# Wionerlol/MultimodalEmotionRecognition

Hardware: AMD Instinct MI355X
Metric: 3s-clip train steps/sec (B=32, xattn fusion) at 1/2/4/8 MI355X (higher is better)
Workload: dtype bf16; 1 GPU; ResNet18 + WavLM-base (frozen) + xattn fusion train step (fwd+bwd+Adam); per_gpu_batch=32, global_batch=32, frames=8, image=112, audio_samples=48000, parallelism=dp1

## Files before the change

### include/mer.h

```cpp
#ifndef MER_H_
#define MER_H_

#define MER_BN_STAT_PARTS 64
#define MER_BN_STAT_ROWS(M) (((M) + 63) / 64 + 64)
#define MER_BN_RED_ROWS(M) (((M) + 63) / 64 + 4 + 64)
#define MER_BN_RED_WS_ROWS 576

#ifdef __cplusplus
extern "C" {
#endif


int mer_gemm_f32(int M, int N, int K, const void* A, int a_dtype, long sam, long sak, long bsa, const void* B,
                 int b_dtype, long sbk, long sbn, long bsb, float* C, long ldc, long bsc, const float* bias, int beta,
                 int act, int splitk, int batch, float* workspace, void* stream);

#define MER_COLSUM_WS_FLOATS(M, N) ((long)(((M) + 15) / 16) * (N))
int mer_colsum_f32(int M, int N, const float* X, long ldx, float* out, float* workspace, void* stream);

int mer_mha_fwd(int B, int H, int Lq, int Lk, int dh, const float* Q, long ldq, const float* K, long ldk,
                const float* V, long ldv, const float* bias, float* O, long ldo, float* P, float scale, float drop_p,
                const unsigned long long* seed, unsigned long long site, void* stream);

int mer_mha_bwd(int B, int H, int Lq, int Lk, int dh, const float* Q, long ldq, const float* K, long ldk,
// ... 32 lines not shown
int mer_softmax_dropout_bwd(int B, int H, int h, int Lq, int Lk, const float* P, const float* dPp, float* dS,
                            float* Pd, float p, const unsigned long long* seed, unsigned long long site, void* stream);
int mer_softmax_dropout_fwd(int B, int H, int h, int Lq, int Lk, const float* S, float scale, float* P, float* Pd,
                            float p, const unsigned long long* seed, unsigned long long site, void* stream);

int mer_cross_entropy(int B, int C, const float* logits, const long long* labels, float label_smoothing, int late,
                      float* loss, float* dlogits, long long* preds, void* stream);

int mer_rng_advance(unsigned long long* state, void* stream);

int mer_scale_dev(long n, const float* x, const float* s, float* y, void* stream);

int mer_dropout_inplace(int rows, int cols, float* x, long ldx, float p, const unsigned long long* seed, unsigned long long site, void* stream);

int mer_relu_dropout_bwd(int rows, int cols, float* dy, long lddy, const float* y, long ldy, float p,
                         const unsigned long long* seed, unsigned long long site, void* stream);

int mer_gate_mix_fwd(int B, int D, const float* z, const float* v, long ldv, const float* a, long lda, float* out,
                     float* g_out, void* stream);
int mer_gate_mix_bwd(int B, int D, const float* g, const float* v, long ldv, const float* a, long lda,
                     const float* dout, float* dz, float* dv, long lddv, float* da, long ldda, void* stream);

int mer_token_bias_fwd(int B, int Lq, int Lk, const float* qt, const float* qp, const float* kt, const float* kp,
                       const float* scale, float* out, void* stream);
int mer_token_bias_bwd(int B, int Lq, int Lk, const float* qt, const float* qp, const float* kt, const float* kp,
                       const float* scale, const float* dbias, float* dqt, float* dkt, float* dqp, float* dkp,
                       float* dscale_part, void* stream);

int mer_softmax_avg_fwd(int B, int C, const float* za, const float* zv, float* out, float* pa, float* pv, void* stream);
int mer_softmax_avg_bwd(int B, int C, const float* pa, const float* pv, const float* dout, float* da, float* dv,
                        void* stream);

int mer_vec_sum(int n, const float* x, float* out, int accumulate, void* stream);

int mer_adam_step(long n, float* p, const float* g, float* m, float* v, float lr, float b1, float b2, float eps,
                  float wd, int step, float grad_scale, void* stream);


int mer_gemm_bf16(int M, int N, int K, const void* A, long a_gstride, long a_rstride, int a_rpg, const void* W,
                  long ldw, void* C, int c_dtype, long ldc, const float* bias, const void* R, long ldr, int act,
                  void* stream);

int mer_gemm_bf16_ex(int M, int N, int K, const void* A, long a_gstride, long a_rstride, int a_rpg, const void* W,
                     long ldw, void* C, int c_dtype, long ldc, const float* bias, const void* R, long ldr, int act,
                     int variant, void* stream);

int mer_posconv_gemm_bf16(int B, int L, int C_total, int groups, int taps, int pad, const void* X, long ldx,
                          const void* Wp, void* out, int out_dtype, long ldo, const float* bias, const void* R,
                          long ldr, int act, int variant, void* stream);

int mer_wavlm_conv0_gn_gelu(int B, int S, int Lout, const float* wav, const float* w0, const float* gamma,
                            const float* beta, float eps, float* workspace, void* out, void* stream);

int mer_layernorm(int rows, int d, const void* x, int x_dtype, long ldx, const float* gamma, const float* beta,
                  float eps, void* y, int y_dtype, long ldy, void* stream);

int mer_wavlm_attention(int B, int L, int H, const void* qkv, long ldqkv, const void* x, long ldx, const float* gate_w,
                        const float* gate_b, const float* gate_const, const float* rel_emb, const int* bucket,
                        void* out, long ldo, float scale, void* stream);

int mer_permute3_bf16(int n0, int n1, int n2, const float* src, long s0, long s1, long s2, const float* scale,
                      void* dst, void* stream);

int mer_weightnorm_scale(int n01, int taps, const float* v, const float* g, float* scale, void* stream);

int mer_cast_bf16(long n, const float* x, void* y, void* stream);


int mer_gemm_bf16_tr(int M, int N, int K, const void* A, long a_gstride, long a_rstride, int a_rpg, const void* W,
                     long ldw, void* C, int c_dtype, long ldc, const float* bias, const void* R, long ldr, int act,
                     float drop_p, const unsigned long long* seed, unsigned long long site, const long long* skip_mask,
                     int skip_bit, int variant, void* stream);

int mer_layernorm_tr(int rows, int d, const void* x, int x_dtype, long ldx, const float* gamma, const float* beta,
                     float eps, void* y, int y_dtype, long ldy, float drop_p, const unsigned long long* seed,
                     unsigned long long site, const long long* skip_mask, int skip_bit, void* stream);

int mer_wavlm_attention_tr(int B, int L, int H, const void* qkv, long ldqkv, const void* x, long ldx,
                           const float* gate_w, const float* gate_b, const float* gate_const, const float* rel_emb,
                           const int* bucket, void* out, long ldo, float scale, float drop_p,
                           const unsigned long long* seed, unsigned long long site, const long long* skip_mask,
                           int skip_bit, void* stream);

int mer_wavlm_time_mask(int B, int L, int D, void* h, long ldh, const float* embed, float mask_prob, int mask_len,
                        int min_masks, const unsigned long long* seed, unsigned long long site, unsigned char* mask_out,
                        void* stream);

int mer_bf16_convert(long n, const void* x, void* y, int y_dtype, void* stream);


int mer_ln_bwd(int rows, int d, const float* dy_a, const float* dy_b, const float* dy_c, const float* x,
               const float* gamma, float eps, float* dx32, void* dx16, float* part, void* stream);

int mer_fold_rows(int parts, int n, const float* part, long ldp, float* out, float* workspace, void* stream);

int mer_colpart(int rows, int cols, const void* x, int x_dtype, long ldx, float* part, void* stream);

int mer_gelu_bf16(long n, const void* z, void* f, void* stream);

int mer_gelu_bwd(int rows, int cols, const float* df, const void* z, void* dz, float* part, void* stream);

int mer_linear_wgrad(int M, int N, int K, const void* x, const void* dy, long ldy, float* dw, int splits,
                     float* workspace, void* stream);

int mer_wavlm_attention_bwd(int B, int L, int H, const void* qkv, long ldqkv, const void* x, long ldx,
                            const void* dout, long ldo, const float* gate_w, const float* gate_b,
                            const float* gate_const, const float* tbl, float scale, void* scratch,
                            void* dqkv, long lddq, float* dx_gate, long lddxg, float* gate_part, void* stream);
int mer_wavlm_attention_bwd_tr(int B, int L, int H, const void* qkv, long ldqkv, const void* x, long ldx,
                               const void* dout, long ldo, const float* gate_w, const float* gate_b,
                               const float* gate_const, const float* tbl, float scale, void* scratch,
                               void* dqkv, long lddq, float* dx_gate, long lddxg, float* gate_part, float drop_p,
                               const unsigned long long* seed, unsigned long long site, void* stream);
int mer_dropout_rows(int rows, int cols, const void* x, int x_dtype, long ldx, float* y32, long ldy32, void* y16,
                     long ldy16, float p, const unsigned long long* seed, unsigned long long site, void* stream);
int mer_wavlm_attention_bwd_kp(int L);

int mer_transpose_bf16(int rows, int cols, const void* src, long lds, void* dst, long ldd, void* stream);


int mer_frames_resize_normalize(int N, int H0, int W0, const void* frames, long frame_stride, int S, float mean0,
                                float mean1, float mean2, float std0, float std1, float std2, float* out, void* stream);

int mer_frames_resize_u8(int N, int H0, int W0, const void* frames, long frame_stride, int S, void* out, void* stream);
int mer_frames_augment_normalize(int N, int S, int T, const void* frames_u8, const float* clip_params,
                                 const unsigned long long* clip_seeds, const float* ztable, float mean0, float mean1,
                                 float mean2, float std0, float std1, float std2, float* out, void* stream);

int mer_wav_pad_crop(int B, int target, const float* packed, const long long* offsets, const long long* lengths,
                     float* out, void* stream);


int mer_conv_fwd(int N, int H, int W, int C, int K, int R, int S, int stride, int pad, const void* x,
                 const void* w_packed, void* y, float* stats, void* stream);

int mer_conv_fwd_ex(int N, int H, int W, int C, int K, int R, int S, int stride, int pad, const void* x,
                    const void* w_packed, void* y, float* stats, int variant, void* stream);

int mer_conv_dgrad(int N, int H, int W, int C, int K, int R, int S, int stride, int pad, const void* dy,
                   const void* wt_packed, void* dx, const void* residual, const void* residual_mask, void* stream);
int mer_conv_dgrad_ex(int N, int H, int W, int C, int K, int R, int S, int stride, int pad, const void* dy,
                      const void* wt_packed, void* dx, const void* residual, const void* residual_mask, int variant,
                      void* stream);

int mer_conv_dgrad_bnr(int N, int H, int W, int C, int K, int R, int S, int stride, int pad, const void* dy,
                       const void* wt_packed, void* dx, const void* residual, const void* residual_mask,
                       const void* bn_mask, const void* bn_x, const float* bn_ms, float* bn_red, const void* bn_x2,
                       const float* bn_ms2, float* bn_red2, int variant, void* stream);
int mer_conv_dgrad_ds(int N, int H, int W, int C, int K, int R, int S, int stride, int pad, const void* dy,
                      const void* wt_packed, void* dx, const void* residual, const void* residual_mask,
                      const void* bn_mask, const void* bn_x, const float* bn_ms, float* bn_red, const void* bn_x2,
                      const float* bn_ms2, float* bn_red2, const void* ds_dy, const void* ds_wt_packed, int ds_K,
                      int variant, void* stream);

int mer_conv_fwd_rows(int N, int H, int W, int C, int K, int R, int S, int stride, int pad, const void* x,
                      const void* w_packed, int variant);
int mer_conv_dgrad_rows(int N, int H, int W, int C, int K, int R, int S, int stride, int pad, const void* dy,
                        const void* wt_packed, const void* ds_dy, int variant);

int mer_partials_sum(int C, int parts, float* in, float* out, void* stream);
int mer_partials_sum2(int C, int parts, float* in, float* out, float* in2, float* out2, void* stream);

int mer_conv_wgrad(int N, int H, int W, int C, int Creal, int K, int R, int S, int stride, int pad, const void* x,
                   const void* dy, float* dw, int splits, float* workspace, void* stream);
int mer_conv_wgrad_ex(int N, int H, int W, int C, int Creal, int K, int R, int S, int stride, int pad, const void* x,
                      const void* dy, float* dw, int splits, float* workspace, int variant, void* stream);
int mer_conv_wgrad_partials(int N, int H, int W, int C, int K, int R, int S, int stride, int pad, const void* x,
                            const void* dy, int splits, float* workspace, int variant, void* stream);
int mer_wgrad_fold_batch(int n, const long long* rows, void* stream);

int mer_pack_input_nhwc(int N, int C, int H, int W, int Cp, const float* x, void* y, void* stream);
int mer_pack_input_s2d(int N, int C, int H, int W, const float* x, void* y, void* stream);

int mer_pack_conv_weight(int K, int C, int R, int S, int Cp, int transpose, const float* w, void* out, void* stream);

int mer_pack_conv_weights(int n, const long long* desc, long total, void* stream);
int mer_pack_conv_weights_flat(int n, const long long* desc, long total_blocks, void* stream);

int mer_bn_finalize(int C, long M, const float* stats, float eps, float momentum, float* ms, float* rmean,
                    float* rvar, long long* num_batches_tracked, void* stream);
int mer_bn_finalize_rows(int C, long M, int data_rows, const float* stats, float eps, float momentum, float* ms,
                         float* rmean, float* rvar, long long* num_batches_tracked, void* stream);
int mer_bn_finalize_rows2(int C, long M, int data_rows, const float* stats, float* ms, float* rmean, float* rvar,
                          long long* nbt, int C2, long M2, int data_rows2, const float* stats2, float* ms2,
                          float* rmean2, float* rvar2, long long* nbt2, float eps, float momentum, void* stream);

int mer_bn_apply(long M, int C, const void* x, const float* ms, const float* gamma, const float* beta, const void* res,
                 const float* ms2, const float* gamma2, const float* beta2, int relu, void* y, void* stream);

int mer_bn_bwd_reduce(long M, int C, const void* dy, const void* mask, const void* x, const float* ms, float* red,
                      float* workspace, void* stream);

int mer_bn_bwd_apply(long M, int C, const void* dy, const void* mask, const void* x, const float* ms,
                     const float* gamma, const float* red, int batch_stats, void* dx, float* dgamma, float* dbeta,
                     void* stream);
int mer_bn_bwd_apply2(long M, int C, const void* dy, const void* mask, const void* x, const float* ms,
                      const float* gamma, const float* red, const void* x2, const float* ms2, const float* gamma2,
                      const float* red2, int batch_stats, void* dx, void* dx2, float* dgamma, float* dbeta,
                      float* dgamma2, float* dbeta2, void* stream);

int mer_stem_bnrelu_maxpool_fwd(int N, int H, int W, int C, const void* x, const float* ms, const float* gamma,
                                const float* beta, void* y, void* argmax, void* stream);
int mer_stem_pool_bn_bwd(int N, int H, int W, int C, const void* dy, const void* argmax, const void* x,
                         const float* ms, const float* gamma, const float* beta, float* red, int batch_stats,
                         void* dx, float* dgamma, float* dbeta, float* workspace, void* stream);

int mer_maxpool_fwd(int N, int H, int W, int C, const void* x, void* y, void* argmax, void* stream);
int mer_maxpool_bwd(int N, int H, int W, int C, const void* dy, const void* argmax, void* dx, void* stream);

int mer_avgpool_fwd(int N, int HW, int C, const void* x, float* y, void* stream);
int mer_avgpool_bwd(int N, int HW, int C, const float* dy, void* dx, void* stream);


int mer_quant_params(long n, const void* x, int x_dtype, float* partial, int mode, float* qparams, void* stream);

int mer_quantize_weight_s8(int N, int K, const float* w, long ldw, const float* qparams, void* qw, long ldq,
                           int* colsum, void* stream);

int mer_gemm_i8dyn(int M, int N, int K, const void* x, int x_dtype, long ldx, const float* x_qparams, const void* qw,
                   long ldq, const float* w_qparams, const int* colsum, const float* bias, int act, float* out, long ldo,
                   void* stream);

int mer_concat_prior_rows(int B, int L, int d, int pd, int ldo, const float* tok, const float* prior, float* out,
                          void* stream);


int mer_xh_split(int n_items, const long long* desc, void* stream);

int mer_xh_audio_fwd_pair(int M, const float* pair, long ldp, const float* bs, const void* Wa_hi, const void* Wa_lo,
                          const float* ba, const void* Wc_hi, const void* Wc_lo, const float* bq2, const float* bkv1,
                          float* a_s, float* a, float* q2, float* kv1, int Mv, int vdim, const float* vfeat,
                          const void* Wv_hi, const void* Wv_lo, const float* bv, const void* Wq1_hi, const void* Wq1_lo,
                          const float* bq1, float* v, float* q1, void* stream);

int mer_xh_audio_fwd(int M, int S, const void* aseq, int aseq_dtype, long ldas, const void* Ws_hi, const void* Ws_lo,
                     const float* bs, const void* Wa_hi, const void* Wa_lo, const float* ba, const void* Wc_hi,
                     const void* Wc_lo, const float* bq2, const float* bkv1, float* a_s, float* a, float* q2,
                     float* kv1, int Mv, int vdim, const float* vfeat, const void* Wv_hi, const void* Wv_lo,
                     const float* bv, const void* Wq1_hi, const void* Wq1_lo, const float* bq1, float* v, float* q1,
                     void* stream);

int mer_xh_v2a_fwd(int B, int T, int Ta, const float* v, const float* q1, const float* kv1, const void* Wo1_hi,
                   const void* Wo1_lo, const float* bo1, const float* gamma, const float* beta, const void* Wkv2_hi,
                   const void* Wkv2_lo, const float* bkv2, float attn_p, float path_p, const unsigned long long* seed,
                   unsigned long long site_attn, unsigned long long site_path, float scale, float* P1, float* o1,
                   float* s_v, float* mean_v, float* rstd_v, float* v1, float* kv2, float* emb, long ld_emb,
                   const float* bias, void* stream);

int mer_xh_a2v_fwd(int B, int T, int Ta, const float* q2, const float* kv2, const float* a, const void* Wo2_hi,
                   const void* Wo2_lo, const float* bo2, const float* gamma, const float* beta, float attn_p,
                   float path_p, const unsigned long long* seed, unsigned long long site_attn,
                   unsigned long long site_path, float scale, float* P2, float* o2, float* s_a, float* mean_a,
                   float* rstd_a, float* part, const float* bias, void* stream);

int mer_xh_prior_fwd(int B, int T, int Ta, int d, int H1, int PD, const float* v, const float* a, const float* W0,
                     const float* b0, const float* W3, const float* b3, const float* w_vq, const float* b_vq,
                     const float* w_ak, const float* b_ak, const float* w_aq, const float* b_aq, const float* w_vk,
                     const float* b_vk, const float* scale, float drop_p, const unsigned long long* seed,
                     unsigned long long site, float* pg, float* h1, float* prior, float* tt_vq, float* tt_ak,
                     float* tt_aq, float* tt_vk, float* tp_vq, float* tp_ak, float* tp_aq, float* tp_vk,
                     float* v2a_bias, float* a2v_bias, void* stream);

int mer_xh_prior_bwd(int B, int T, int Ta, int d, int H1, int PD, const float* dbias_v2a, const float* dbias_a2v,
                     const float* tt_vq, const float* tt_ak, const float* tt_aq, const float* tt_vk,
                     const float* tp_vq, const float* tp_ak, const float* tp_aq, const float* tp_vk,
                     const float* scale, const float* w_vq, const float* w_ak, const float* w_aq, const float* w_vk,
                     const float* W0, const float* W3, const float* h1, float drop_p, const unsigned long long* seed,
                     unsigned long long site, float* dtt_vq, float* dtt_ak, float* dtt_aq, float* dtt_vk,
                     float* dtp_vq, float* dtp_ak, float* dtp_aq, float* dtp_vk, float* dprior, float* dh1,
                     float* dscale_part, float* dv, float* da, void* stream);

int mer_xh_mlp_fwd(int B, int Ta, int gated, int H1, int C, const float* part, float* emb, const float* W0,
                   const float* b0, const float* W3, const float* b3, const float* Wc, const float* bc, float mlp_p,
                   const unsigned long long* seed, unsigned long long site, float* hsave, float* gsave, float* fsave,
                   float* logits, void* stream);


int mer_xh_mlp_bwd(int B, int C, int H1, int gated, const float* dlogits, const float* emb, const float* h,
                   const float* g, const float* W0, const float* W3, const float* Wc, float mlp_p,
                   const unsigned long long* seed, unsigned long long site, float* dh, float* dz, float* demb,
                   void* stream);

int mer_xh_a2v_bwd(int B, int T, int Ta, const float* demb, const float* s_a, const float* mean_a, const float* rstd_a,
                   const float* gamma, const float* P2, const float* kv2, const float* q2, const void* WoT2_hi,
                   const void* WoT2_lo, float attn_p, float path_p, const unsigned long long* seed,
                   unsigned long long site_attn, unsigned long long site_path, float scale, float* da, float* da2,
                   float* dqkv, float* dkv2_part, float* ln_part, float* dbias, void* stream);

int mer_xh_v2a_bwd(int B, int T, int Ta, const float* dkv2_part, const void* WkvT2_hi, const void* WkvT2_lo,
                   const float* demb, const float* s_v, const float* mean_v, const float* rstd_v, const float* gamma,
                   const void* WoT1_hi, const void* WoT1_lo, const float* P1, const float* kv1, const float* q1,
                   float attn_p, float path_p, const unsigned long long* seed, unsigned long long site_attn,
                   unsigned long long site_path, float scale, float* dkv2, float* dv2, float* dq1, float* dv,
                   float* dqkv, float* ln_part, float* do1, float* dS_heads, float* dbias, void* stream);

int mer_xh_audio_bwd(int M, const float* dqkv, const void* WcT_hi, const void* WcT_lo, const void* WaT_hi,
                     const void* WaT_lo, float* da, float* da_s, int Mv, int vdim, const float* dq1,
                     const void* WqT1_hi, const void* WqT1_lo, const void* WvT_hi, const void* WvT_lo, float* dv,
                     float* dvfeat, void* stream);

int mer_xh_wgrad_ws_floats(int nprob, const long long* table, long long* out);
int mer_xh_wgrad(int nprob, const long long* table, float* ws, long long ws_floats, void* stream);

int mer_clip_align_fwd(int B, int D, const float* a, const float* v, const float* log_scale, float* an, float* vn,
                       float* norms, float* logits, float* loss, void* stream);
int mer_clip_align_bwd(int B, int D, const float* an, const float* vn, const float* norms, const float* logits,
                       const float* log_scale, const float* dloss, float* ws, float* da, float* dv, float* dlog_scale,
                       void* stream);
int mer_add_scaled_scalar(const float* x, const float* y, float w, float* out, void* stream);

#ifdef __cplusplus
}
#endif
#endif
```

### multimodalemotionrecognition_amd/csrc/bn_pool.hip

```cpp
#include "common.h"
#include "mer.h"

typedef __attribute__((ext_vector_type(4))) uint32_t u32x4;

__global__ __launch_bounds__(256) void bn_stat_rows_fold_kernel(int C2, int rows, int per, const float* __restrict__ in,
                                                                float* __restrict__ out) {
  __shared__ float part[4][64];
  const int el = threadIdx.x & 63, pg = threadIdx.x >> 6;
  const int e = blockIdx.x * 64 + el, grp = blockIdx.y;
  const int r0 = grp * per, r1 = min(rows, r0 + per);
  const int ec = e < C2 ? e : C2 - 1;
  const int n = r1 - (r0 + pg) > 0 ? (r1 - (r0 + pg) + 3) / 4 : 0;
  float a0 = 0.f, a1 = 0.f;
  for (int i0 = 0; i0 < n; i0 += 16) {
    float x[16];
#pragma unroll
    for (int i = 0; i < 16; ++i) {
      const int r = r0 + pg + 4 * (i0 + i);
      x[i] = in[(long)(r < r1 ? r : r1 - 1) * C2 + ec];
    }
#pragma unroll
    for (int i = 0; i < 16; i += 2) {
      if (i0 + i < n) a0 += x[i];
      if (i0 + i + 1 < n) a1 += x[i + 1];
// ... 435 lines not shown
  hipLaunchKernelGGL(partials_sum_kernel, dim3((2 * C + 63) / 64), dim3(256), 0, st, C, parts, src, out);
  MER_LAUNCH_CHECK();
}
MER_API int mer_partials_sum(int C, int parts, float* in, float* out, void* stream) {
  if (C <= 0 || parts <= 0) return (int)hipErrorInvalidValue;
  return partials_fold(C, parts, in, out, (hipStream_t)stream);
}

MER_API int mer_partials_sum2(int C, int parts, float* in, float* out, float* in2, float* out2, void* stream) {
  if (C <= 0 || parts <= 0 || !in || !out || !in2 || !out2) return (int)hipErrorInvalidValue;
  hipStream_t st = (hipStream_t)stream;
  if (parts > BN_WIDE_ROWS) {
    const int rc = partials_fold(C, parts, in, out, st);
    return rc ? rc : partials_fold(C, parts, in2, out2, st);
  }
  const dim3 grid((2 * C + 63) / 64, 2);
#define MER_PSUM2(NB) \
  [&] { hipLaunchKernelGGL(partials_sum_wide2_kernel<NB>, grid, dim3(1024), 0, st, 2 * C, parts, in, out, in2, out2); }
  wide_pick(parts, MER_PSUM2(16), MER_PSUM2(32), MER_PSUM2(64));
#undef MER_PSUM2
  MER_LAUNCH_CHECK();
}

template <bool BNMASK>
__global__ __launch_bounds__(256) void bn_bwd_apply_kernel(long M, int C, const bf16_t* dy,
                                                           const bf16_t* __restrict__ mask,
                                                           const bf16_t* __restrict__ x, const float* __restrict__ ms,
                                                           const float* __restrict__ gamma,
                                                           const float* __restrict__ mbeta,
                                                           const float* __restrict__ red, int batch_stats,
                                                           bf16_t* dx, float* __restrict__ dgamma,
                                                           float* __restrict__ dbeta) {
  __shared__ __attribute__((aligned(16))) float coef[5][512];
  const float invM = 1.f / (float)M;
  for (int c = threadIdx.x; c < C; c += 256) {
    if (blockIdx.x == 0) {
      if (dgamma) dgamma[c] += red[2 * c + 1];
      if (dbeta) dbeta[c] += red[2 * c];
    }
    const float mu = ms[2 * c], rs = ms[2 * c + 1], gr = gamma[c] * rs;
    const float a = batch_stats ? red[2 * c] * invM : 0.f;
    const float b = batch_stats ? red[2 * c + 1] * invM : 0.f;
    const float t = gr * b * rs;
    coef[0][c] = gr;
    coef[1][c] = -t;
    coef[2][c] = fmaf(-gr, a, t * mu);
    if (BNMASK) stem_bn_coef(c, ms, gamma, mbeta, coef[3][c], coef[4][c]);
  }
  __syncthreads();
  const long nvec = M * C / 8;
  const long stride = (long)gridDim.x * blockDim.x;
  const long tid0 = blockIdx.x * (long)blockDim.x + threadIdx.x;
  const int c0 = (int)(tid0 % (C / 8)) * 8;
  float k1[8], k2[8], k0[8], msc[8], msh[8];
#pragma unroll
  for (int i = 0; i < 8; ++i) {
    k1[i] = coef[0][c0 + i];
    k2[i] = coef[1][c0 + i];
    k0[i] = coef[2][c0 + i];
    msc[i] = BNMASK ? coef[3][c0 + i] : 0.f;
    msh[i] = BNMASK ? coef[4][c0 + i] : 0.f;
  }
  auto one = [&](const u32x4& gv, const u32x4& xv, const u32x4& mv) -> u32x4 {
    const bf16_t* gh = reinterpret_cast<const bf16_t*>(&gv);
    const bf16_t* xh = reinterpret_cast<const bf16_t*>(&xv);
    const bf16_t* mh = reinterpret_cast<const bf16_t*>(&mv);
    u32x4 ov;
    bf16_t* oh = reinterpret_cast<bf16_t*>(&ov);
#pragma unroll
    for (int i = 0; i < 8; ++i) {
      const bool live = BNMASK ? bf2f(f2bf(fmaxf(bf2f(xh[i]) * msc[i] + msh[i], 0.f))) > 0.f
                               : (!mask || bf2f(mh[i]) > 0.f);
      const float g = live ? bf2f(gh[i]) : 0.f;
      oh[i] = f2bf(fmaf(k1[i], g, fmaf(k2[i], bf2f(xh[i]), k0[i])));
    }
    return ov;
  };
  const u32x4 one16 = {0x3f803f80u, 0x3f803f80u, 0x3f803f80u, 0x3f803f80u};
  long e = tid0;
  for (; e + stride < nvec; e += 2 * stride) {
    const long e1 = e + stride;
    const u32x4 g0 = *reinterpret_cast<const u32x4*>(dy + e * 8);
    const u32x4 g1 = *reinterpret_cast<const u32x4*>(dy + e1 * 8);
    const u32x4 x0 = *reinterpret_cast<const u32x4*>(x + e * 8);
    const u32x4 x1 = *reinterpret_cast<const u32x4*>(x + e1 * 8);
    const u32x4 m0 = (!BNMASK && mask) ? *reinterpret_cast<const u32x4*>(mask + e * 8) : one16;
    const u32x4 m1 = (!BNMASK && mask) ? *reinterpret_cast<const u32x4*>(mask + e1 * 8) : one16;
    *reinterpret_cast<u32x4*>(dx + e * 8) = one(g0, x0, m0);
    *reinterpret_cast<u32x4*>(dx + e1 * 8) = one(g1, x1, m1);
  }
  if (e < nvec) {
    const u32x4 g0 = *reinterpret_cast<const u32x4*>(dy + e * 8);
    const u32x4 x0 = *reinterpret_cast<const u32x4*>(x + e * 8);
    const u32x4 m0 = (!BNMASK && mask) ? *reinterpret_cast<const u32x4*>(mask + e * 8) : one16;
    *reinterpret_cast<u32x4*>(dx + e * 8) = one(g0, x0, m0);
  }
}
MER_API int mer_bn_bwd_apply(long M, int C, const void* dy, const void* mask, const void* x, const float* ms,
                             const float* gamma, const float* red, int batch_stats, void* dx, float* dgamma,
                             float* dbeta, void* stream) {
  if (C % 8 || C > 512 || 256 % (C / 8)) return (int)hipErrorInvalidValue;
  const long nvec = M * C / 8;
  const int grid = bn_stream_grid(nvec);
  hipLaunchKernelGGL((bn_bwd_apply_kernel<false>), dim3(grid), dim3(256), 0, (hipStream_t)stream, M, C,
                     (const bf16_t*)dy, (const bf16_t*)mask, (const bf16_t*)x, ms, gamma, (const float*)nullptr, red,
                     batch_stats, (bf16_t*)dx, dgamma, dbeta);
  MER_LAUNCH_CHECK();
}

__global__ __launch_bounds__(256) void bn_bwd_apply2_kernel(long M, int C, const bf16_t* __restrict__ dy,
                                                            const bf16_t* __restrict__ mask,
                                                            const bf16_t* __restrict__ x, const float* __restrict__ ms,
                                                            const float* __restrict__ gamma,
                                                            const float* __restrict__ red,
                                                            const bf16_t* __restrict__ x2,
                                                            const float* __restrict__ ms2,
                                                            const float* __restrict__ gamma2,
                                                            const float* __restrict__ red2, int batch_stats,
                                                            bf16_t* __restrict__ dx, bf16_t* __restrict__ dx2,
                                                            float* __restrict__ dgamma, float* __restrict__ dbeta,
                                                            float* __restrict__ dgamma2, float* __restrict__ dbeta2) {
  __shared__ __attribute__((aligned(16))) float coef[6][512];
  const float invM = 1.f / (float)M;
  for (int c = threadIdx.x; c < C; c += 256) {
#pragma unroll
    for (int h = 0; h < 2; ++h) {
      const float* rd = h ? red2 : red;
      const float* m = h ? ms2 : ms;
      if (blockIdx.x == 0) {
        float* dg = h ? dgamma2 : dgamma;
        float* db = h ? dbeta2 : dbeta;
        if (dg) dg[c] += rd[2 * c + 1];
        if (db) db[c] += rd[2 * c];
      }
      const float mu = m[2 * c], rs = m[2 * c + 1], gr = (h ? gamma2 : gamma)[c] * rs;
      const float a = batch_stats ? rd[2 * c] * invM : 0.f;
      const float b = batch_stats ? rd[2 * c + 1] * invM : 0.f;
      const float t = gr * b * rs;
      coef[3 * h + 0][c] = gr;
      coef[3 * h + 1][c] = -t;
      coef[3 * h + 2][c] = fmaf(-gr, a, t * mu);
    }
  }
  __syncthreads();
  const long nvec = M * C / 8;
  const long stride = (long)gridDim.x * blockDim.x;
  const long tid0 = blockIdx.x * (long)blockDim.x + threadIdx.x;
  const int c0 = (int)(tid0 % (C / 8)) * 8;
  float k[6][8];
#pragma unroll
  for (int j = 0; j < 6; ++j)
#pragma unroll
    for (int i = 0; i < 8; ++i) k[j][i] = coef[j][c0 + i];
  for (long e = tid0; e < nvec; e += stride) {
    const u32x4 gv = *reinterpret_cast<const u32x4*>(dy + e * 8);
    const u32x4 mv = *reinterpret_cast<const u32x4*>(mask + e * 8);
    const u32x4 xv = *reinterpret_cast<const u32x4*>(x + e * 8);
    const u32x4 x2v = *reinterpret_cast<const u32x4*>(x2 + e * 8);
    const bf16_t* gh = reinterpret_cast<const bf16_t*>(&gv);
    const bf16_t* mh = reinterpret_cast<const bf16_t*>(&mv);
    const bf16_t* xh = reinterpret_cast<const bf16_t*>(&xv);
    const bf16_t* x2h = reinterpret_cast<const bf16_t*>(&x2v);
    u32x4 ov, o2v;
    bf16_t* oh = reinterpret_cast<bf16_t*>(&ov);
    bf16_t* o2h = reinterpret_cast<bf16_t*>(&o2v);
#pragma unroll
    for (int i = 0; i < 8; ++i) {
      const float g = bf2f(mh[i]) > 0.f ? bf2f(gh[i]) : 0.f;
      oh[i] = f2bf(fmaf(k[0][i], g, fmaf(k[1][i], bf2f(xh[i]), k[2][i])));
      o2h[i] = f2bf(fmaf(k[3][i], g, fmaf(k[4][i], bf2f(x2h[i]), k[5][i])));
    }
    *reinterpret_cast<u32x4*>(dx + e * 8) = ov;
    *reinterpret_cast<u32x4*>(dx2 + e * 8) = o2v;
  }
}
MER_API int mer_bn_bwd_apply2(long M, int C, const void* dy, const void* mask, const void* x, const float* ms,
                              const float* gamma, const float* red, const void* x2, const float* ms2,
                              const float* gamma2, const float* red2, int batch_stats, void* dx, void* dx2,
                              float* dgamma, float* dbeta, float* dgamma2, float* dbeta2, void* stream) {
  if (C % 8 || C > 512 || 256 % (C / 8) || !mask || !x2 || !dx2 || dx == dy || dx2 == dy)
    return (int)hipErrorInvalidValue;
  const long nvec = M * C / 8;
  const int grid = bn_stream_grid(nvec);
  hipLaunchKernelGGL(bn_bwd_apply2_kernel, dim3(grid), dim3(256), 0, (hipStream_t)stream, M, C, (const bf16_t*)dy,
                     (const bf16_t*)mask, (const bf16_t*)x, ms, gamma, red, (const bf16_t*)x2, ms2, gamma2, red2,
                     batch_stats, (bf16_t*)dx, (bf16_t*)dx2, dgamma, dbeta, dgamma2, dbeta2);
  MER_LAUNCH_CHECK();
}

__global__ void maxpool_fwd_kernel(int N, int H, int W, int C, int Ho, int Wo, const bf16_t* __restrict__ x,
                                   bf16_t* __restrict__ y, uint8_t* __restrict__ arg) {
  const int cpr = C / 8;
  const int total = N * Ho * Wo * cpr;
  const float inv_cpr = 1.f / cpr, inv_Wo = 1.f / Wo, inv_Ho = 1.f / Ho;
  for (int e = blockIdx.x * blockDim.x + threadIdx.x; e < total; e += gridDim.x * blockDim.x) {
    const int q = fdiv(e, inv_cpr);
    const int c0 = (e - q * cpr) * 8;
    const int q2 = fdiv(q, inv_Wo);
    const int ow = q - q2 * Wo;
    const int n = fdiv(q2, inv_Ho);
    const int oh = q2 - n * Ho;
    float best[8];
    int bi[8];
#pragma unroll
    for (int i = 0; i < 8; ++i) { best[i] = -INFINITY; bi[i] = 0; }
    for (int r = 0; r < 3; ++r)
      for (int s = 0; s < 3; ++s) {
        const int ih = oh * 2 - 1 + r, iw = ow * 2 - 1 + s;
        if (ih < 0 || ih >= H || iw < 0 || iw >= W) continue;
        const u32x4 v = *reinterpret_cast<const u32x4*>(x + (((long)n * H + ih) * W + iw) * C + c0);
        const bf16_t* vh = reinterpret_cast<const bf16_t*>(&v);
#pragma unroll
        for (int i = 0; i < 8; ++i) {
          const float f = bf2f(vh[i]);
          if (f > best[i]) { best[i] = f; bi[i] = r * 3 + s; }
        }
      }
    u32x4 o;
    bf16_t* oh8 = reinterpret_cast<bf16_t*>(&o);
    uint2 a;
    uint8_t* a8 = reinterpret_cast<uint8_t*>(&a);
#pragma unroll
    for (int i = 0; i < 8; ++i) { oh8[i] = f2bf(best[i]); a8[i] = (uint8_t)bi[i]; }
    *reinterpret_cast<u32x4*>(y + (long)q * C + c0) = o;
    *reinterpret_cast<uint2*>(arg + (long)q * C + c0) = a;
  }
}
MER_API int mer_maxpool_fwd(int N, int H, int W, int C, const void* x, void* y, void* argmax, void* stream) {
  const int Ho = (H + 2 - 3) / 2 + 1, Wo = (W + 2 - 3) / 2 + 1;
  if (C % 8 || (long)N * H * W >= (1L << 22)) return (int)hipErrorInvalidValue;
  const long total = (long)N * Ho * Wo * C / 8;
  const int grid = (int)((total + 255) / 256 < 8192 ? (total + 255) / 256 : 8192);
  hipLaunchKernelGGL(maxpool_fwd_kernel, dim3(grid), dim3(256), 0, (hipStream_t)stream, N, H, W, C, Ho, Wo,
                     (const bf16_t*)x, (bf16_t*)y, (uint8_t*)argmax);
  MER_LAUNCH_CHECK();
}
__global__ void maxpool_bwd_kernel(int N, int H, int W, int C, int Ho, int Wo, const bf16_t* __restrict__ dy,
                                   const uint8_t* __restrict__ arg, bf16_t* __restrict__ dx) {
  const int cpr = C / 8;
  const int total = N * H * W * cpr;
  const float inv_cpr = 1.f / cpr, inv_W = 1.f / W, inv_H = 1.f / H;
  for (int e = blockIdx.x * blockDim.x + threadIdx.x; e < total; e += gridDim.x * blockDim.x) {
    const int q = fdiv(e, inv_cpr);
    const int c0 = (e - q * cpr) * 8;
    const int q2 = fdiv(q, inv_W);
    const int w = q - q2 * W;
    const int n = fdiv(q2, inv_H);
    const int h = q2 - n * H;
    float acc[8] = {0.f, 0.f, 0.f, 0.f, 0.f, 0.f, 0.f, 0.f};
    u32x4 gq[2][2];
    uint2 aq[2][2];
    int tap[2][2];
#pragma unroll
    for (int a = 0; a < 2; ++a)
#pragma unroll
      for (int b = 0; b < 2; ++b) {
        const int oh = (h + 1) / 2 - 1 + a, ow = (w + 1) / 2 - 1 + b;
        const int r = h - (oh * 2 - 1), s = w - (ow * 2 - 1);
        const bool ok = oh >= 0 && oh < Ho && ow >= 0 && ow < Wo && r >= 0 && r <= 2 && s >= 0 && s <= 2;
        const int ohc = oh < 0 ? 0 : (oh >= Ho ? Ho - 1 : oh), owc = ow < 0 ? 0 : (ow >= Wo ? Wo - 1 : ow);
        const long oi = (((long)n * Ho + ohc) * Wo + owc) * C + c0;
        gq[a][b] = *reinterpret_cast<const u32x4*>(dy + oi);
        aq[a][b] = *reinterpret_cast<const uint2*>(arg + oi);
        tap[a][b] = ok ? r * 3 + s : -1;
      }
#pragma unroll
    for (int a = 0; a < 2; ++a)
#pragma unroll
      for (int b = 0; b < 2; ++b) {
        const bf16_t* gh = reinterpret_cast<const bf16_t*>(&gq[a][b]);
        const uint8_t* a8 = reinterpret_cast<const uint8_t*>(&aq[a][b]);
#pragma unroll
        for (int i = 0; i < 8; ++i)
          if ((int)a8[i] == tap[a][b]) acc[i] += bf2f(gh[i]);
      }
    u32x4 o;
    bf16_t* oh8 = reinterpret_cast<bf16_t*>(&o);
#pragma unroll
    for (int i = 0; i < 8; ++i) oh8[i] = f2bf(acc[i]);
    *reinterpret_cast<u32x4*>(dx + (long)q * C + c0) = o;
  }
}
MER_API int mer_maxpool_bwd(int N, int H, int W, int C, const void* dy, const void* argmax, void* dx, void* stream) {
  const int Ho = (H + 2 - 3) / 2 + 1, Wo = (W + 2 - 3) / 2 + 1;
  if (C % 8 || (long)N * H * W >= (1L << 22)) return (int)hipErrorInvalidValue;
  const long total = (long)N * H * W * C / 8;
  const int grid = (int)((total + 255) / 256 < 8192 ? (total + 255) / 256 : 8192);
  hipLaunchKernelGGL(maxpool_bwd_kernel, dim3(grid), dim3(256), 0, (hipStream_t)stream, N, H, W, C, Ho, Wo,
                     (const bf16_t*)dy, (const uint8_t*)argmax, (bf16_t*)dx);
  MER_LAUNCH_CHECK();
}


__global__ void stem_bnrelu_maxpool_kernel(int N, int H, int W, int C, int Ho, int Wo, const bf16_t* __restrict__ x,
                                           const float* __restrict__ ms, const float* __restrict__ gamma,
                                           const float* __restrict__ beta, bf16_t* __restrict__ y,
                                           uint8_t* __restrict__ arg) {
  const int cpr = C / 8;
  const int total = N * Ho * Wo * cpr;
  const float inv_cpr = 1.f / cpr, inv_Wo = 1.f / Wo, inv_Ho = 1.f / Ho;
  for (int e = blockIdx.x * blockDim.x + threadIdx.x; e < total; e += gridDim.x * blockDim.x) {
    const int q = fdiv(e, inv_cpr);
    const int c0 = (e - q * cpr) * 8;
    const int q2 = fdiv(q, inv_Wo);
    const int ow = q - q2 * Wo;
    const int n = fdiv(q2, inv_Ho);
    const int oh = q2 - n * Ho;
    float sc[8], sh[8], best[8];
    int bi[8];
#pragma unroll
    for (int i = 0; i < 8; ++i) {
      stem_bn_coef(c0 + i, ms, gamma, beta, sc[i], sh[i]);
      best[i] = -INFINITY;
      bi[i] = 0;
    }
    u32x4 v[9];
#pragma unroll
    for (int t = 0; t < 9; ++t) {
      const int ih = oh * 2 - 1 + t / 3, iw = ow * 2 - 1 + t % 3;
      const int ihc = ih < 0 ? 0 : (ih >= H ? H - 1 : ih), iwc = iw < 0 ? 0 : (iw >= W ? W - 1 : iw);
      v[t] = *reinterpret_cast<const u32x4*>(x + (((long)n * H + ihc) * W + iwc) * C + c0);
    }
#pragma unroll
    for (int t = 0; t < 9; ++t) {
      const int ih = oh * 2 - 1 + t / 3, iw = ow * 2 - 1 + t % 3;
      const bool ok = ih >= 0 && ih < H && iw >= 0 && iw < W;
      const bf16_t* vh = reinterpret_cast<const bf16_t*>(&v[t]);
#pragma unroll
      for (int i = 0; i < 8; ++i) {
        const float f = ok ? bf2f(f2bf(fmaxf(bf2f(vh[i]) * sc[i] + sh[i], 0.f))) : -INFINITY;
        if (f > best[i]) { best[i] = f; bi[i] = t; }
      }
    }
    u32x4 o;
    bf16_t* oh8 = reinterpret_cast<bf16_t*>(&o);
    uint2 a;
    uint8_t* a8 = reinterpret_cast<uint8_t*>(&a);
#pragma unroll
    for (int i = 0; i < 8; ++i) { oh8[i] = f2bf(best[i]); a8[i] = (uint8_t)bi[i]; }
    *reinterpret_cast<u32x4*>(y + (long)q * C + c0) = o;
    *reinterpret_cast<uint2*>(arg + (long)q * C + c0) = a;
  }
}

MER_API int mer_stem_bnrelu_maxpool_fwd(int N, int H, int W, int C, const void* x, const float* ms, const float* gamma,
                                        const float* beta, void* y, void* argmax, void* stream) {
  const int Ho = (H + 2 - 3) / 2 + 1, Wo = (W + 2 - 3) / 2 + 1;
  if (C % 8 || C > 512 || (long)N * H * W >= (1L << 22)) return (int)hipErrorInvalidValue;
  const long total = (long)N * Ho * Wo * C / 8;
  const int grid = (int)((total + 255) / 256 < 8192 ? (total + 255) / 256 : 8192);
  hipLaunchKernelGGL(stem_bnrelu_maxpool_kernel, dim3(grid), dim3(256), 0, (hipStream_t)stream, N, H, W, C, Ho, Wo,
                     (const bf16_t*)x, ms, gamma, beta, (bf16_t*)y, (uint8_t*)argmax);
  MER_LAUNCH_CHECK();
}

MER_API int mer_stem_pool_bn_bwd(int N, int H, int W, int C, const void* dy, const void* argmax, const void* x,
                                 const float* ms, const float* gamma, const float* beta, float* red, int batch_stats,
                                 void* dx, float* dgamma, float* dbeta, float* workspace, void* stream) {
  if (C % 8 || C > 512 || 256 % (C / 8) || (long)N * H * W >= (1L << 22)) return (int)hipErrorInvalidValue;
  const hipStream_t st = (hipStream_t)stream;
  const long M = (long)N * H * W;
  int rc = mer_maxpool_bwd(N, H, W, C, dy, argmax, dx, stream);
  if (rc) return rc;
  const long rpb = bn_bwd_reduce_rpb(M);
  const int blocks = (int)((M + rpb - 1) / rpb);
  hipLaunchKernelGGL((bn_bwd_reduce_kernel<true>), dim3((unsigned)blocks), dim3(256), 0, st, M, C, (const bf16_t*)dx,
                     (const bf16_t*)nullptr, (const bf16_t*)x, ms, gamma, beta, workspace, rpb);
  rc = partials_fold(C, blocks, workspace, red, st);
  if (rc) return rc;
  hipLaunchKernelGGL((bn_bwd_apply_kernel<true>), dim3(bn_stream_grid(M * C / 8)), dim3(256), 0, st, M, C,
                     (const bf16_t*)dx, (const bf16_t*)nullptr, (const bf16_t*)x, ms, gamma, beta, red, batch_stats,
                     (bf16_t*)dx, dgamma, dbeta);
  MER_LAUNCH_CHECK();
}

__global__ void avgpool_fwd_kernel(int N, int HW, int C, const bf16_t* __restrict__ x, float* __restrict__ y) {
  const int n = blockIdx.y, c = blockIdx.x * blockDim.x + threadIdx.x;
  if (c >= C) return;
  float s = 0.f;
  for (int p = 0; p < HW; ++p) s += bf2f(x[((long)n * HW + p) * C + c]);
  y[(long)n * C + c] = s / HW;
}
__global__ void avgpool_bwd_kernel(int N, int HW, int C, const float* __restrict__ dy, bf16_t* __restrict__ dx) {
  const int n = blockIdx.y;
  for (int e = blockIdx.x * blockDim.x + threadIdx.x; e < HW * C; e += gridDim.x * blockDim.x) {
    const int c = e % C;
    dx[(long)n * HW * C + e] = f2bf(dy[(long)n * C + c] / HW);
  }
}
MER_API int mer_avgpool_fwd(int N, int HW, int C, const void* x, float* y, void* stream) {
  hipLaunchKernelGGL(avgpool_fwd_kernel, dim3((C + 255) / 256, N), dim3(256), 0, (hipStream_t)stream, N, HW, C,
                     (const bf16_t*)x, y);
  MER_LAUNCH_CHECK();
}
MER_API int mer_avgpool_bwd(int N, int HW, int C, const float* dy, void* dx, void* stream) {
  dim3 grid((HW * C + 255) / 256, N);
  hipLaunchKernelGGL(avgpool_bwd_kernel, grid, dim3(256), 0, (hipStream_t)stream, N, HW, C, dy, (bf16_t*)dx);
  MER_LAUNCH_CHECK();
}
```

### multimodalemotionrecognition_amd/csrc/conv.hip

```cpp
#include "conv_common.h"
#include "mer.h"

MER_CT_BUFFER(mer_ct, 512 * 64)
MER_CT_BUFFER(mer_ctp, 4096 * 8)
#define CT(k) CT_AT(mer_ct_buf, k)
#define CTP(k) CTP_AT(mer_ctp_buf, k)

namespace {

template <bool DGRAD>
__device__ __forceinline__ u32x4 conv_a_chunk(const ConvGeom& g, int n, int oh, int ow, bool rowok, int kk, int tap,
                                              int c, int r, int s) {
  u32x4 v = {0u, 0u, 0u, 0u};
  if (!rowok || kk >= g.Kred) return v;
  int ih, iw;
  if (!DGRAD) {
    ih = oh * g.st - g.pad + r;
    iw = ow * g.st - g.pad + s;
  } else {
    const int th = oh + g.pad - r, tw = ow + g.pad - s;
    if (th < 0 || tw < 0) return v;
    if (g.st == 1) {
      ih = th;
      iw = tw;
// ... 171 lines not shown

__device__ __forceinline__ ParClass par_class(const ConvGeom& g, int cls) {
  ParClass c;
  c.ph = cls >> 1;
  c.pw = cls & 1;
  c.Hc = (g.OH - c.ph + 1) >> 1;
  c.Wc = (g.OW - c.pw + 1) >> 1;
  c.r0 = (c.ph + g.pad) & 1;
  c.s0 = (c.pw + g.pad) & 1;
  c.nr = (g.R - c.r0 + 1) >> 1;
  c.ns = (g.S - c.s0 + 1) >> 1;
  c.dh0 = (c.ph + g.pad - c.r0) >> 1;
  c.dw0 = (c.pw + g.pad - c.s0) >> 1;
  return c;
}

template <int FM, int FN, int WM, int WN>
__device__ __forceinline__ void conv_tile_stats_lane(const ConvGeom& g, const f32x4 (&acc)[FM][FN], int w, int lane,
                                                     int m0, int n0, int M, float (&part)[FN][2]) {
  constexpr int TM = FM * 16, TN = FN * 16;
  const int wr = w / WN, wc = w % WN, fr = lane & 15, fq = lane >> 4;
#pragma unroll
  for (int j = 0; j < FN; ++j) {
    const int col = n0 + wc * TN + j * 16 + fr;
    float csum = 0.f, csq = 0.f;
#pragma unroll
    for (int i = 0; i < FM; ++i)
#pragma unroll
      for (int r = 0; r < 4; ++r) {
        const int row = m0 + wr * TM + i * 16 + fq * 4 + r;
        if (row < M && col < g.Ncols) {
          const float hv = acc[i][j][r];
          csum += hv;
          csq += hv * hv;
        }
      }
    part[j][0] = csum;
    part[j][1] = csq;
  }
}

template <int FN, int WM, int WN>
__device__ __forceinline__ void conv_stats_finish(const ConvGeom& g, float (&part)[FN][2], float* red, int w, int lane,
                                                  int n0, long stat_row) {
  constexpr int TN = FN * 16;
  const int wr = w / WN, wc = w % WN, fr = lane & 15, fq = lane >> 4;
#pragma unroll
  for (int j = 0; j < FN; ++j)
#pragma unroll
    for (int q = 0; q < 2; ++q) {
      part[j][q] += __shfl_xor(part[j][q], 16, 64);
      part[j][q] += __shfl_xor(part[j][q], 32, 64);
    }
  lds_barrier();
  if (wr > 0 && fq == 0)
#pragma unroll
    for (int j = 0; j < FN; ++j) {
      red[((wr * WN + wc) * FN * 16 + j * 16 + fr) * 2] = part[j][0];
      red[((wr * WN + wc) * FN * 16 + j * 16 + fr) * 2 + 1] = part[j][1];
    }
  lds_barrier();
  if (wr == 0 && fq == 0) {
    float* slab = g.stats + stat_row * g.Ncols * 2;
#pragma unroll
    for (int j = 0; j < FN; ++j) {
      const int col = n0 + wc * TN + j * 16 + fr;
      float t0 = part[j][0], t1 = part[j][1];
#pragma unroll
      for (int q = 1; q < WM; ++q) {
        t0 += red[((q * WN + wc) * FN * 16 + j * 16 + fr) * 2];
        t1 += red[((q * WN + wc) * FN * 16 + j * 16 + fr) * 2 + 1];
      }
      if (col < g.Ncols) {
        slab[2 * col] = t0;
        slab[2 * col + 1] = t1;
      }
    }
  }
}

template <int FM, int FN, int WM, int WN>
__device__ __forceinline__ void conv_tile_stats(const ConvGeom& g, const f32x4 (&acc)[FM][FN], float* red, int w,
                                                int lane, int m0, int n0, int M, long stat_row) {
  float part[FN][2];
  conv_tile_stats_lane<FM, FN, WM, WN>(g, acc, w, lane, m0, n0, M, part);
  conv_stats_finish<FN, WM, WN>(g, part, red, w, lane, n0, stat_row);
}

typedef __attribute__((ext_vector_type(8))) float f32x8;
template <int FN>
struct EpiAcc {
  f32x8 sA, sB, sC;
  float fs[FN][2];
  __device__ void zero() {
    sA = sB = sC = f32x8{0.f, 0.f, 0.f, 0.f, 0.f, 0.f, 0.f, 0.f};
#pragma unroll
    for (int j = 0; j < FN; ++j) fs[j][0] = fs[j][1] = 0.f;
  }
};
struct EpiNoAcc {};

template <int FM, int FN, int WAVE_FLOATS>
struct EpiGeo {
  static constexpr int TM = FM * 16, TN = FN * 16, LDT = TN + 4;
  static constexpr int GI0 = WAVE_FLOATS / (16 * LDT);
  static constexpr int GI = GI0 < FM ? GI0 : FM;
  static constexpr int LPR = TN / 8, RPP = 64 / LPR;
  static constexpr int PPG = (GI * 16 + RPP - 1) / RPP;
  static constexpr int NP = ((FM + GI - 1) / GI) * PPG;
};

template <int NP>
struct EpiPre {
  u32x4 r[NP], m[NP], bm[NP], x[NP], x2[NP];
  float mu[8], rs[8], mu2[8], rs2[8];
};
struct EpiNone {};

template <bool DGRAD, int FM, int FN, int WM, int WN, int WAVE_FLOATS, class OutRow, int NP, bool X2 = true>
__device__ __forceinline__ void conv_epilogue_prefetch(const ConvGeom& g, EpiPre<NP>& pre, int w, int lane, int m0,
                                                       int n0, int M, OutRow out_row) {
  using E = EpiGeo<FM, FN, WAVE_FLOATS>;
  static_assert(NP == E::NP, "prefetch pass count");
  const int wr = w / WN, wc = w % WN;
  const int lr = lane / E::LPR, lc = (lane % E::LPR) * 8;
  const int colv = n0 + wc * E::TN + lc;
  const bool cok = colv < g.Ncols;
  const bool do_bnr = DGRAD && g.bnr_red != nullptr;
  const bool has_x2 = X2 && do_bnr && g.bnr_x2 != nullptr;
  const u32x4 z = {0u, 0u, 0u, 0u};
#pragma unroll
  for (int e = 0; e < 8; ++e) {
    const int col = cok ? colv + e : 0;
    pre.mu[e] = do_bnr ? g.bnr_ms[2 * col] : 0.f;
    pre.rs[e] = do_bnr ? g.bnr_ms[2 * col + 1] : 0.f;
    pre.mu2[e] = has_x2 ? g.bnr_ms2[2 * col] : 0.f;
    pre.rs2[e] = has_x2 ? g.bnr_ms2[2 * col + 1] : 0.f;
  }
#pragma unroll
  for (int q = 0; q < NP; ++q) {
    const int i0 = (q / E::PPG) * E::GI, rr = (q % E::PPG) * E::RPP;
    int row = m0 + wr * E::TM + i0 * 16 + rr + lr;
    row = row < M ? row : M - 1;
    const long e0 = out_row(row) * g.ldy + (cok ? colv : 0);
    pre.r[q] = (DGRAD && g.R_) ? *reinterpret_cast<const u32x4*>(g.R_ + e0) : z;
    pre.m[q] = (DGRAD && g.R_ && g.Rmask) ? *reinterpret_cast<const u32x4*>(g.Rmask + e0) : z;
    pre.bm[q] = do_bnr ? *reinterpret_cast<const u32x4*>(g.bnr_mask + e0) : z;
    pre.x[q] = do_bnr ? *reinterpret_cast<const u32x4*>(g.bnr_x + e0) : z;
    pre.x2[q] = has_x2 ? *reinterpret_cast<const u32x4*>(g.bnr_x2 + e0) : z;
  }
}

template <bool DGRAD, int FM, int FN, int WM, int WN, int WAVE_FLOATS, class OutRow, class Pre = EpiNone,
          bool DEFER = false, bool X2 = true, class AccT = EpiNoAcc>
__device__ __forceinline__ void conv_epilogue_vec(const ConvGeom& g, f32x4 (&acc)[FM][FN], float* smemf, int w,
                                                  int lane, int m0, int n0, int M, long red_row_id, long stat_row,
                                                  OutRow out_row, const Pre* pre = nullptr, int ct_slot = -1,
                                                  AccT* accp = nullptr) {
  constexpr bool PREF = !std::is_same<Pre, EpiNone>::value;
  constexpr bool ACC = !std::is_same<AccT, EpiNoAcc>::value;
  using E = EpiGeo<FM, FN, WAVE_FLOATS>;
  constexpr int TM = FM * 16, TN = FN * 16;
  const int wr = w / WN, wc = w % WN, fr = lane & 15, fq = lane >> 4;
  constexpr int LDT = TN + 4;
  constexpr int GI = E::GI;
  static_assert(GI >= 1, "epilogue staging slice too small");
  constexpr int LPR = TN / 8, RPP = 64 / LPR;
  float* wl = smemf + w * WAVE_FLOATS;
  const int lr = lane / LPR, lc = (lane % LPR) * 8;
  const int colv = n0 + wc * TN + lc;
  const bool cok = colv < g.Ncols;
  const bool do_bnr = DGRAD && g.bnr_red != nullptr;
  const bool has_x2 = X2 && do_bnr && g.bnr_x2 != nullptr;
  float mu[8], rs[8], mu2[8], rs2[8];
  float sA[8], sB[8], sC[8];
  constexpr int NPS = DEFER ? E::NP : 1;
  u32x4 pend[NPS];
  long pend_at[NPS];
  bool pend_ok[NPS];
#pragma unroll
  for (int q = 0; q < NPS; ++q) pend_ok[q] = false;
  auto flush = [&]() {
#pragma unroll
    for (int q = 0; q < NPS; ++q)
      if (pend_ok[q]) *reinterpret_cast<u32x4*>(g.Y + pend_at[q]) = pend[q];
  };
#pragma unroll
  for (int e = 0; e < 8; ++e) {
    if constexpr (PREF) {
      mu[e] = pre->mu[e];
      rs[e] = pre->rs[e];
      mu2[e] = pre->mu2[e];
      rs2[e] = pre->rs2[e];
    } else {
      const int col = cok ? colv + e : 0;
      mu[e] = do_bnr ? g.bnr_ms[2 * col] : 0.f;
      rs[e] = do_bnr ? g.bnr_ms[2 * col + 1] : 0.f;
      mu2[e] = has_x2 ? g.bnr_ms2[2 * col] : 0.f;
      rs2[e] = has_x2 ? g.bnr_ms2[2 * col + 1] : 0.f;
    }
    sA[e] = sB[e] = sC[e] = 0.f;
  }
#pragma unroll
  for (int i0 = 0; i0 < FM; i0 += GI) {
#pragma unroll
    for (int ii = 0; ii < GI; ++ii) {
      if (i0 + ii >= FM) break;
#pragma unroll
      for (int j = 0; j < FN; ++j)
#pragma unroll
        for (int r = 0; r < 4; ++r) wl[(ii * 16 + fq * 4 + r) * LDT + j * 16 + fr] = acc[i0 + ii][j][r];
    }
    __builtin_amdgcn_fence(__ATOMIC_RELEASE, "wavefront");
    __builtin_amdgcn_wave_barrier();
    __builtin_amdgcn_fence(__ATOMIC_ACQUIRE, "wavefront");
    const int nrows = (FM - i0 < GI ? FM - i0 : GI) * 16;
#pragma unroll
    for (int rr = 0; rr < GI * 16; rr += RPP) {
      const int rl = rr + lr;
      const int row = m0 + wr * TM + i0 * 16 + rl;
      if (rl < nrows && row < M && cok) {
        const f32x4 lo = *reinterpret_cast<const f32x4*>(&wl[rl * LDT + lc]);
        const f32x4 hi = *reinterpret_cast<const f32x4*>(&wl[rl * LDT + lc + 4]);
        float v[8] = {lo[0], lo[1], lo[2], lo[3], hi[0], hi[1], hi[2], hi[3]};
        const long e0 = out_row(row) * g.ldy + colv;
        const int q = (i0 / GI) * E::PPG + rr / RPP;
        if (DGRAD && g.R_) {
          u32x4 rv, mv;
          if constexpr (PREF) {
            rv = pre->r[q];
            mv = g.Rmask ? pre->m[q] : u32x4{1u, 1u, 1u, 1u};
          } else {
            rv = *reinterpret_cast<const u32x4*>(g.R_ + e0);
            mv = g.Rmask ? *reinterpret_cast<const u32x4*>(g.Rmask + e0) : u32x4{1u, 1u, 1u, 1u};
          }
          const bf16_t* rh = reinterpret_cast<const bf16_t*>(&rv);
          const bf16_t* mh = reinterpret_cast<const bf16_t*>(&mv);
#pragma unroll
          for (int e = 0; e < 8; ++e)
            if (!g.Rmask || bf2f(mh[e]) > 0.f) v[e] += bf2f(rh[e]);
        }
        u32x4 ov;
        bf16_t* oh = reinterpret_cast<bf16_t*>(&ov);
#pragma unroll
        for (int e = 0; e < 8; ++e) {
          oh[e] = f2bf(v[e]);
          v[e] = bf2f(oh[e]);
        }
        if constexpr (DEFER) {
          pend[q] = ov;
          pend_at[q] = e0;
          pend_ok[q] = true;
        } else {
          *reinterpret_cast<u32x4*>(g.Y + e0) = ov;
        }
        if (do_bnr) {
          u32x4 mv, xv, x2v;
          if constexpr (PREF) {
            mv = pre->bm[q];
            xv = pre->x[q];
            x2v = pre->x2[q];
          } else {
            mv = *reinterpret_cast<const u32x4*>(g.bnr_mask + e0);
            xv = *reinterpret_cast<const u32x4*>(g.bnr_x + e0);
            x2v = has_x2 ? *reinterpret_cast<const u32x4*>(g.bnr_x2 + e0) : u32x4{0u, 0u, 0u, 0u};
          }
          const bf16_t* mh = reinterpret_cast<const bf16_t*>(&mv);
          const bf16_t* xh = reinterpret_cast<const bf16_t*>(&xv);
          const bf16_t* x2h = reinterpret_cast<const bf16_t*>(&x2v);
#pragma unroll
          for (int e = 0; e < 8; ++e) {
            const float gv = bf2f(mh[e]) > 0.f ? v[e] : 0.f;
            sA[e] += gv;
            sB[e] += gv * (bf2f(xh[e]) - mu[e]) * rs[e];
            if (has_x2) sC[e] += gv * (bf2f(x2h[e]) - mu2[e]) * rs2[e];
          }
        }
      }
    }
    __builtin_amdgcn_fence(__ATOMIC_RELEASE, "wavefront");
    __builtin_amdgcn_wave_barrier();
    __builtin_amdgcn_fence(__ATOMIC_ACQUIRE, "wavefront");
  }
  if (ct_slot >= 0) CT(ct_slot);
  if constexpr (ACC) {
    if (do_bnr) {
#pragma unroll
      for (int e = 0; e < 8; ++e) {
        accp->sA[e] += sA[e];
        accp->sB[e] += sB[e];
        accp->sC[e] += sC[e];
      }
      flush();
      return;
    }
  }
  if (do_bnr) {
#pragma unroll
  for (int o = LPR; o < 64; o <<= 1)
#pragma unroll
    for (int e = 0; e < 8; ++e) {
      sA[e] += __shfl_xor(sA[e], o, 64);
      sB[e] += __shfl_xor(sB[e], o, 64);
      if (has_x2) sC[e] += __shfl_xor(sC[e], o, 64);
    }
  if (ct_slot >= 0) CT(ct_slot + 3);
  float* red = smemf;
  lds_barrier();
  if (ct_slot >= 0) CT(ct_slot + 4);
  if (wr > 0 && lane < LPR)
#pragma unroll
    for (int e = 0; e < 8; ++e) {
      float* o = red + ((wr * WN + wc) * TN + lc + e) * 3;
      o[0] = sA[e];
      o[1] = sB[e];
      o[2] = sC[e];
    }
  lds_barrier();
  if (wr != 0 || lane >= LPR || !cok) {
    flush();
    return;
  }
#pragma unroll
  for (int e = 0; e < 8; ++e)
#pragma unroll
    for (int q = 1; q < WM; ++q) {
      const float* o = red + ((q * WN + wc) * TN + lc + e) * 3;
      sA[e] += o[0];
      sB[e] += o[1];
      sC[e] += o[2];
    }
  {
    const long slab = red_row_id * g.Ncols * 2 + 2 * colv;
#pragma unroll
    for (int e = 0; e < 8; e += 2) {
      *reinterpret_cast<f32x4*>(g.bnr_red + slab + 2 * e) = f32x4{sA[e], sB[e], sA[e + 1], sB[e + 1]};
      if (g.bnr_red2)
        *reinterpret_cast<f32x4*>(g.bnr_red2 + slab + 2 * e) = f32x4{sA[e], sC[e], sA[e + 1], sC[e + 1]};
    }
  }
  if (ct_slot >= 0) CT(ct_slot + 1);
  flush();
  if (ct_slot >= 0) CT(ct_slot + 2);
  return;
  }
  if (!g.stats) {
    flush();
    return;
  }
#pragma unroll
  for (int i = 0; i < FM; ++i)
#pragma unroll
    for (int j = 0; j < FN; ++j)
#pragma unroll
      for (int r = 0; r < 4; ++r) acc[i][j][r] = bf2f(f2bf(acc[i][j][r]));
  if constexpr (ACC) {
    float part[FN][2];
    conv_tile_stats_lane<FM, FN, WM, WN>(g, acc, w, lane, m0, n0, M, part);
#pragma unroll
    for (int j = 0; j < FN; ++j) {
      accp->fs[j][0] += part[j][0];
      accp->fs[j][1] += part[j][1];
    }
    flush();
    return;
  }
  conv_tile_stats<FM, FN, WM, WN>(g, acc, smemf, w, lane, m0, n0, M, stat_row);
  if (ct_slot >= 0) CT(ct_slot + 1);
  flush();
  if (ct_slot >= 0) CT(ct_slot + 2);
}

template <bool DGRAD, int FM, int FN, int WM, int WN, int WAVE_FLOATS, bool X2 = true>
__device__ __forceinline__ void conv_epilogue_acc_finish(const ConvGeom& g, EpiAcc<FN>& a, float* smemf, int w,
                                                         int lane, int n0, long row_id) {
  if constexpr (DGRAD) {
    if (!g.bnr_red) return;
    using E = EpiGeo<FM, FN, WAVE_FLOATS>;
    constexpr int TN = FN * 16, LPR = E::LPR;
    const int wr = w / WN, wc = w % WN;
    const int lc = (lane % LPR) * 8;
    const int colv = n0 + wc * TN + lc;
    const bool cok = colv < g.Ncols;
    const bool has_x2 = X2 && g.bnr_x2 != nullptr;
#pragma unroll
    for (int o = LPR; o < 64; o <<= 1)
#pragma unroll
      for (int e = 0; e < 8; ++e) {
        a.sA[e] += __shfl_xor(a.sA[e], o, 64);
        a.sB[e] += __shfl_xor(a.sB[e], o, 64);
        if (has_x2) a.sC[e] += __shfl_xor(a.sC[e], o, 64);
      }
    float* red = smemf;
    lds_barrier();
    if (wr > 0 && lane < LPR)
#pragma unroll
      for (int e = 0; e < 8; ++e) {
        float* o = red + ((wr * WN + wc) * TN + lc + e) * 3;
        o[0] = a.sA[e];
        o[1] = a.sB[e];
        o[2] = a.sC[e];
      }
    lds_barrier();
    if (wr != 0 || lane >= LPR || !cok) return;
#pragma unroll
    for (int e = 0; e < 8; ++e)
#pragma unroll
      for (int q = 1; q < WM; ++q) {
        const float* o = red + ((q * WN + wc) * TN + lc + e) * 3;
        a.sA[e] += o[0];
        a.sB[e] += o[1];
        a.sC[e] += o[2];
      }
    const long slab = row_id * g.Ncols * 2 + 2 * colv;
#pragma unroll
    for (int e = 0; e < 8; e += 2) {
      *reinterpret_cast<f32x4*>(g.bnr_red + slab + 2 * e) = f32x4{a.sA[e], a.sB[e], a.sA[e + 1], a.sB[e + 1]};
      if (g.bnr_red2)
        *reinterpret_cast<f32x4*>(g.bnr_red2 + slab + 2 * e) = f32x4{a.sA[e], a.sC[e], a.sA[e + 1], a.sC[e + 1]};
    }
  } else {
    if (!g.stats) return;
    conv_stats_finish<FN, WM, WN>(g, a.fs, smemf, w, lane, n0, row_id);
  }
}

constexpr int conv_pipe_wpe(int nw, int bm, int bn, int stages, bool dgrad, bool par, int lds_bytes = 0) {
  return (nw >= 16 || 2 * lds_bytes > 160 * 1024)
             ? (nw >= 4 ? nw / 4 : 1)
             : nw == 8 ? ((dgrad && (bm == 256 || (!par && bm == 128 && bn == 128 && stages == 3))) ? 2 : 4) : 2;
}
constexpr int conv_pipe_lds(int bm, int bn, int stages, int ks, int kg) {
  return kg * stages * (bm + bn) * ks * 2 > (kg > 1 ? kg * bm * (bn + 4) * 4 : 0)
             ? kg * stages * (bm + bn) * ks * 2
             : kg * bm * (bn + 4) * 4;
}

template <int BM_, int BN_, int NW>
struct KgLayout {
  static constexpr int WM = (NW >= 4 && BM_ / 4 >= 16) ? 4 : (NW >= 2 ? 2 : 1);
  static constexpr int WN = NW / WM;
  static_assert(WM * WN == NW && BM_ % (16 * WM) == 0 && BN_ % (16 * WN) == 0, "split-K epilogue layout");
};

template <bool DGRAD, bool PAR, int BM_, int BN_, int WM = 2, int WN = 2, int STAGES = 2, int KS = 64, bool X2 = true,
          int KG = 1, bool FAST = false>
__global__ __launch_bounds__(64 * WM * WN * KG, conv_pipe_wpe(WM * WN * KG, BM_, BN_, STAGES, DGRAD, PAR,
                                                              conv_pipe_lds(BM_, BN_, STAGES, KS, KG))) void conv_pipe_kernel(ConvGeom g) {
  constexpr int WAVES = WM * WN;
  constexpr int CW = KS / 8, RPG = 64 / CW;
  constexpr int IA = BM_ / RPG / WAVES, IB = BN_ / RPG / WAVES;
  static_assert(IA * RPG * WAVES == BM_ && IB * RPG * WAVES == BN_, "tile rows must split into whole glds pieces");
  static_assert(KS == 64 || KS == 32, "K-tile");
  static_assert(KG == 1 || KG == 2 || KG == 4, "K-groups");
  constexpr int TM = BM_ / WM, TN = BN_ / WN, FM = TM / 16, FN = TN / 16;
  constexpr int BUF = (BM_ + BN_) * KS;
  extern __shared__ __attribute__((aligned(16))) bf16_t smem_all[];
  const int t = threadIdx.x, lane = t & 63, kg = (t >> 6) / WAVES, w = (t >> 6) % WAVES;
  bf16_t* const smem = smem_all + kg * STAGES * BUF;
  ParClass pc{};
  int M, Kr, rowsH, rowsW;
  int Kr0 = 0;
  if (PAR) {
    pc = par_class(g, par_cls());
    M = g.N * pc.Hc * pc.Wc;
    Kr0 = pc.nr * pc.ns * g.IC;
    Kr = Kr0 + ((g.X2 && pc.ph == 0 && pc.pw == 0) ? g.K2 : 0);
    rowsH = pc.Hc;
    rowsW = pc.Wc;
  } else {
    M = g.N * g.OH * g.OW;
    Kr = g.Kred;
    rowsH = g.OH;
    rowsW = g.OW;
  }
  const int nx = (g.Ncols + BN_ - 1) / BN_, ny = (M + BM_ - 1) / BM_;
  if ((int)blockIdx.x >= nx * ny) return;
  CTP(0);
  int tx, ty;
  xcd_tile(blockIdx.x, nx, nx * ny, tx, ty);
// ... 135 lines not shown
    }
    k_loop([&](int buf) {
      bf16_t* la = smem + buf * BUF;
      bf16_t* lb = la + BM_ * KS;
      const unsigned tbit = 1u << (f_tap & 31);
      const long ao = f_aoff + f_c, bo = f_boff + f_c;
#pragma unroll
      for (int j = 0; j < IA; ++j) glds16((fm[j] & tbit) ? fa[j] + ao : zero, la + (w * IA + j) * 512);
#pragma unroll
      for (int j = 0; j < IB; ++j) glds16(bok[j] ? fb[j] + bo : zero, lb + (w * IB + j) * 512);
      f_c += KS;
      if (f_c == f_ic) {
        f_c = 0;
        ++f_tap;
        if (++f_si == ns) {
          f_si = 0;
          ++f_ri;
        }
        tap_offsets();
        if (has_ds && !f_ds && f_tap == nr * ns) enter_ds();
      }
    });
  } else {
    int an[IA], aoh[IA], aow[IA];
    bool aok[IA];
#pragma unroll
    for (int j = 0; j < IA; ++j) a_row(j, an[j], aoh[j], aow[j], aok[j]);
    const bf16_t* pb[IB];
    const bf16_t* pb2[IB];
#pragma unroll
    for (int j = 0; j < IB; ++j) {
      pb[j] = g.Wt + (long)bn[j] * g.Kred;
      pb2[j] = g.Wt2 + (long)bn[j] * g.K2;
    }
    const float inv_IC = 1.f / g.IC, inv_S = 1.f / g.S, inv_ns = PAR ? 1.f / pc.ns : 1.f;
    auto par_a_src = [&](int n, int hh, int ww, bool rowok, int kk) -> const bf16_t* {
      if (!rowok || kk >= Kr) return zero;
      if (kk >= Kr0)
        return g.X2 + (((long)n * g.IH + hh) * g.IW + ww) * g.K2 + (kk - Kr0);
      const int tap = fdiv(kk, inv_IC), c = kk - tap * g.IC;
      const int ri = fdiv(tap, inv_ns), si = tap - ri * pc.ns;
      const int ih = hh + pc.dh0 - ri, iw = ww + pc.dw0 - si;
      if (ih < 0 || ih >= g.IH || iw < 0 || iw >= g.IW) return zero;
      return g.X + (((long)n * g.IH + ih) * g.IW + iw) * g.IC + c;
    };
    auto par_b_off = [&](int kk) -> int {
      const int tap = fdiv(kk, inv_IC), c = kk - tap * g.IC;
      const int ri = fdiv(tap, inv_ns), si = tap - ri * pc.ns;
      return ((pc.r0 + 2 * ri) * g.S + pc.s0 + 2 * si) * g.IC + c;
    };
    int k0 = kofs;
    k_loop([&](int buf) {
      bf16_t* la = smem + buf * BUF;
      bf16_t* lb = la + BM_ * KS;
#pragma unroll
      for (int j = 0; j < IA; ++j) {
        const bf16_t* src = PAR ? par_a_src(an[j], aoh[j], aow[j], aok[j], k0 + acl[j])
                                : conv_a_src<DGRAD>(g, an[j], aoh[j], aow[j], aok[j], k0 + acl[j], inv_IC, inv_S);
        glds16(src, la + (w * IA + j) * 512);
      }
#pragma unroll
      for (int j = 0; j < IB; ++j) {
        const int kk = k0 + bcl[j];
        const bool ok = bok[j] && kk < Kr;
        const bf16_t* src = !PAR ? pb[j] + kk : (kk >= Kr0 ? pb2[j] + (kk - Kr0) : pb[j] + par_b_off(kk));
        glds16(ok ? src : zero, lb + (w * IB + j) * 512);
      }
      k0 += KS;
    });
  }
  CTP(2);

  auto out_row = [&](int row) -> long {
    if (!PAR) return (long)row;
    const int n = row / (pc.Hc * pc.Wc);
    const int rem = row - n * pc.Hc * pc.Wc;
    const int hh = rem / pc.Wc, ww = rem - hh * pc.Wc;
    return ((long)n * g.OH + 2 * hh + pc.ph) * g.OW + 2 * ww + pc.pw;
  };
  auto red_row = [&]() -> long {
    long row_id = ty;
    if (PAR)
      for (int c2 = 0; c2 < par_cls(); ++c2) {
        const ParClass q = par_class(g, c2);
        row_id += (g.N * q.Hc * q.Wc + BM_ - 1) / BM_;
      }
    return row_id;
  };
  constexpr int EWF = STAGES * BUF / 2 / WAVES;
  const int ct_slot = 10;
  if constexpr (KG > 1) {
    using L = KgLayout<BM_, BN_, WAVES * KG>;
    constexpr int LDR = BN_ + 4;
    constexpr int TM2 = BM_ / L::WM, TN2 = BN_ / L::WN, FM2 = TM2 / 16, FN2 = TN2 / 16;
    using E2 = EpiGeo<FM2, FN2, EWF>;
    const int w2 = t >> 6, wr2 = w2 / L::WN, wc2 = w2 % L::WN;
    constexpr bool PF = DGRAD && E2::NP == 1;
    EpiPre<E2::NP> pre;
    if constexpr (PF)
      conv_epilogue_prefetch<DGRAD, FM2, FN2, L::WM, L::WN, EWF, decltype(out_row), E2::NP, X2>(g, pre, w2, lane, m0,
                                                                                                n0, M, out_row);
    __syncthreads();
    float* const part = reinterpret_cast<float*>(smem_all);
    {
      float* mine = part + kg * BM_ * LDR;
#pragma unroll
      for (int i = 0; i < FM; ++i)
#pragma unroll
        for (int j = 0; j < FN; ++j)
#pragma unroll
          for (int r = 0; r < 4; ++r) mine[(wr * TM + i * 16 + fq * 4 + r) * LDR + wc * TN + j * 16 + fr] = acc[i][j][r];
    }
    lds_barrier();
    f32x4 acc2[FM2][FN2];
#pragma unroll
    for (int i = 0; i < FM2; ++i)
#pragma unroll
      for (int j = 0; j < FN2; ++j)
#pragma unroll
        for (int r = 0; r < 4; ++r) {
          const int e = (wr2 * TM2 + i * 16 + fq * 4 + r) * LDR + wc2 * TN2 + j * 16 + fr;
          float s = part[e];
#pragma unroll
          for (int q = 1; q < KG; ++q) s += part[q * BM_ * LDR + e];
          acc2[i][j][r] = s;
        }
    lds_barrier();
    CTP(3);
    if constexpr (PF)
      conv_epilogue_vec<DGRAD, FM2, FN2, L::WM, L::WN, EWF, decltype(out_row), decltype(pre), false, X2>(
          g, acc2, reinterpret_cast<float*>(smem_all), w2, lane, m0, n0, M, g.bnr_red ? red_row() : 0l, ty, out_row,
          &pre, ct_slot);
    else
      conv_epilogue_vec<DGRAD, FM2, FN2, L::WM, L::WN, EWF, decltype(out_row), EpiNone, false, X2>(
          g, acc2, reinterpret_cast<float*>(smem_all), w2, lane, m0, n0, M, (DGRAD && g.bnr_red) ? red_row() : 0l, ty,
          out_row, static_cast<const EpiNone*>(nullptr), ct_slot);
    CTP(4);
    return;
  }
  if (g.vec) {
    using E1 = EpiGeo<FM, FN, EWF>;
    if constexpr (DGRAD && E1::NP == 1) {
      EpiPre<E1::NP> pre;
      conv_epilogue_prefetch<DGRAD, FM, FN, WM, WN, EWF, decltype(out_row), E1::NP, X2>(g, pre, w, lane, m0, n0, M,
                                                                                         out_row);
      __syncthreads();
      CTP(3);
      conv_epilogue_vec<DGRAD, FM, FN, WM, WN, EWF, decltype(out_row), decltype(pre), false, X2>(
          g, acc, reinterpret_cast<float*>(smem), w, lane, m0, n0, M, g.bnr_red ? red_row() : 0l, ty, out_row, &pre,
          ct_slot);
    } else {
      __syncthreads();
      CTP(3);
      conv_epilogue_vec<DGRAD, FM, FN, WM, WN, EWF, decltype(out_row), EpiNone, false, X2>(
          g, acc, reinterpret_cast<float*>(smem), w, lane, m0, n0, M, (DGRAD && g.bnr_red) ? red_row() : 0l, ty,
          out_row, static_cast<const EpiNone*>(nullptr), ct_slot);
    }
    CTP(4);
    return;
  } else {
  __syncthreads();
#pragma unroll
  for (int i = 0; i < FM; ++i)
#pragma unroll
    for (int r = 0; r < 4; ++r) {
      const int row = m0 + wr * TM + i * 16 + fq * 4 + r;
      if (row >= M) continue;
      const long orow = out_row(row) * g.ldy;
#pragma unroll
      for (int j = 0; j < FN; ++j) {
        const int col = n0 + wc * TN + j * 16 + fr;
        if (col >= g.Ncols) continue;
        float v = acc[i][j][r];
        if (g.R_) {
          const long ri = orow + col;
          if (!g.Rmask || bf2f(g.Rmask[ri]) > 0.f) v += bf2f(g.R_[ri]);
        }
        const bf16_t h = f2bf(v);
        g.Y[orow + col] = h;
        acc[i][j][r] = bf2f(h);
      }
    }
  if (DGRAD && g.bnr_red) {
    float ps[FN][3];
#pragma unroll
    for (int j = 0; j < FN; ++j) {
      const int col = n0 + wc * TN + j * 16 + fr;
      const bool cok = col < g.Ncols;
      const float mu = cok ? g.bnr_ms[2 * col] : 0.f, rs = cok ? g.bnr_ms[2 * col + 1] : 0.f;
      const float mu2 = (cok && g.bnr_x2) ? g.bnr_ms2[2 * col] : 0.f;
      const float rs2 = (cok && g.bnr_x2) ? g.bnr_ms2[2 * col + 1] : 0.f;
      float s1 = 0.f, s2 = 0.f, s3 = 0.f;
#pragma unroll
      for (int i = 0; i < FM; ++i)
#pragma unroll
        for (int r = 0; r < 4; ++r) {
          const int row = m0 + wr * TM + i * 16 + fq * 4 + r;
          if (row < M && cok) {
            const long e = out_row(row) * g.ldy + col;
            const float gv = bf2f(g.bnr_mask[e]) > 0.f ? acc[i][j][r] : 0.f;
            s1 += gv;
            s2 += gv * (bf2f(g.bnr_x[e]) - mu) * rs;
            if (g.bnr_x2) s3 += gv * (bf2f(g.bnr_x2[e]) - mu2) * rs2;
          }
        }
#pragma unroll
      for (int o = 16; o < 64; o <<= 1) {
        s1 += __shfl_xor(s1, o, 64);
        s2 += __shfl_xor(s2, o, 64);
        s3 += __shfl_xor(s3, o, 64);
      }
      ps[j][0] = s1;
      ps[j][1] = s2;
      ps[j][2] = s3;
    }
    float* red = reinterpret_cast<float*>(smem);
    __syncthreads();
    if (wr > 0 && fq == 0)
#pragma unroll
      for (int j = 0; j < FN; ++j)
#pragma unroll
        for (int q = 0; q < 3; ++q) red[((wr * WN + wc) * FN * 16 + j * 16 + fr) * 3 + q] = ps[j][q];
    __syncthreads();
    if (wr == 0 && fq == 0) {
      long row_id = ty;
      if (PAR)
        for (int c2 = 0; c2 < par_cls(); ++c2) {
          const ParClass q = par_class(g, c2);
          row_id += (g.N * q.Hc * q.Wc + BM_ - 1) / BM_;
        }
      const long slab = row_id * g.Ncols * 2;
#pragma unroll
      for (int j = 0; j < FN; ++j) {
        const int col = n0 + wc * TN + j * 16 + fr;
        float t0 = ps[j][0], t1 = ps[j][1], t2 = ps[j][2];
#pragma unroll
        for (int q = 1; q < WM; ++q) {
          const float* o = red + ((q * WN + wc) * FN * 16 + j * 16 + fr) * 3;
          t0 += o[0];
          t1 += o[1];
          t2 += o[2];
        }
        if (col < g.Ncols) {
          g.bnr_red[slab + 2 * col] = t0;
          g.bnr_red[slab + 2 * col + 1] = t1;
          if (g.bnr_red2) {
            g.bnr_red2[slab + 2 * col] = t0;
            g.bnr_red2[slab + 2 * col + 1] = t2;
          }
        }
      }
    }
  }
  }
  if (g.stats) conv_tile_stats<FM, FN, WM, WN>(g, acc, reinterpret_cast<float*>(smem), w, lane, m0, n0, M, ty);
}

template <int BM_, int BN_, int WM_ = 2, int WN_ = 2, int STAGES_ = 2, int KS_ = 64, int KG_ = 1>
struct Tile {
  static constexpr int BM = BM_, BN = BN_, WM = WM_, WN = WN_, STAGES = STAGES_, KS = KS_, KG = KG_;
};

enum ConvFamily { kConvNone, kConvHalo, kConvReg, kConvPipe };

struct ConvPlan {
  int err;
  ConvFamily family;
  int halo;
  int variant;
  bool par;
  int BM, BN, WM, WN, STAGES, KS, KG;
  bool x2, fast;
  size_t lds;
  unsigned grid_x, grid_y;
  int rows;
};

template <bool DGRAD, bool PAR, class T>
int launch_conv_pipe_t(ConvGeom& g, const ConvPlan& p, hipStream_t st) {
  if (T::BM != p.BM || T::BN != p.BN || T::WM != p.WM || T::WN != p.WN || T::STAGES != p.STAGES || T::KS != p.KS ||
      T::KG != p.KG)
    return (int)hipErrorInvalidConfiguration;
  auto launch = [&](void (*kern)(ConvGeom)) -> int {
    if (hipFuncSetAttribute(reinterpret_cast<const void*>(kern), hipFuncAttributeMaxDynamicSharedMemorySize,
                            (int)p.lds) != hipSuccess)
      return (int)hipErrorInvalidConfiguration;
    hipLaunchKernelGGL(kern, dim3(p.grid_x, p.grid_y), dim3(64 * T::WM * T::WN * T::KG), p.lds, st, g);
    return (int)hipGetLastError();
  };
  if constexpr (DGRAD && !PAR) {
    if (!p.x2)
      return p.fast ? launch(&conv_pipe_kernel<DGRAD, PAR, T::BM, T::BN, T::WM, T::WN, T::STAGES, T::KS, false, T::KG,
                                               true>)
                    : launch(&conv_pipe_kernel<DGRAD, PAR, T::BM, T::BN, T::WM, T::WN, T::STAGES, T::KS, false, T::KG,
                                               false>);
  }
  return p.fast
             ? launch(&conv_pipe_kernel<DGRAD, PAR, T::BM, T::BN, T::WM, T::WN, T::STAGES, T::KS, true, T::KG, true>)
             : launch(&conv_pipe_kernel<DGRAD, PAR, T::BM, T::BN, T::WM, T::WN, T::STAGES, T::KS, true, T::KG, false>);
}

inline int conv_bn(const ConvGeom& g) { return g.Ncols <= 64 ? 64 : 128; }
inline bool conv_small_m(const ConvGeom& g, bool par) {
  const long M = (long)g.N * g.OH * g.OW / (par ? 4 : 1);
  const int bn = conv_bn(g);
  return ((M + 127) / 128) * ((g.Ncols + bn - 1) / bn) * (par ? 4 : 1) < 384;
}

template <bool DGRAD, bool PAR, class F>
int conv_pipe_tile(const ConvGeom& g, int variant, F&& f) {
  const int bn = conv_bn(g);
  const bool small_m = conv_small_m(g, PAR);
  if (variant == 7) {
    if (bn == 64) return PAR ? f(Tile<64, 64, 2, 2, 2, 64, 2>{}) : f(Tile<64, 64, 2, 2, 3, 64, 2>{});
    return PAR ? f(Tile<64, 128, 2, 4, 2, 64, 2>{}) : f(Tile<64, 128, 2, 4, 3, 64, 2>{});
  }
  if (variant == 3 && !small_m) {
    if constexpr (DGRAD) {
      return f(Tile<256, 64, 4, 2>{});
    } else {
      if (bn == 64) return f(Tile<256, 64, 4, 2>{});
      return f(Tile<256, 128, 4, 4>{});
    }
  }
  if (variant == 5) {
    if (bn == 64) return small_m ? f(Tile<64, 64, 2, 2, 4, 32>{}) : f(Tile<128, 64, 2, 2, 4, 32>{});
    return small_m ? f(Tile<64, 128, 2, 2, 4, 32>{}) : f(Tile<128, 128, 2, 4, 4, 32>{});
  }
  if (variant == 4) {
    if (bn == 64) return small_m ? f(Tile<64, 64, 2, 2, 3>{}) : f(Tile<128, 64, 4, 2, 3>{});
    return small_m ? f(Tile<64, 128, 2, 4, 3>{}) : f(Tile<128, 128, 2, 4, 3>{});
  }
// ... 220 lines not shown
      const long ntiles = (M + halo::BM - 1) / halo::BM, slots = (long)halo_occ(hk) * cu_count();
      p.family = kConvHalo;
      p.halo = hk;
      p.variant = 6;
      p.BM = halo::BM; p.BN = 64; p.WM = 4; p.WN = 2;
      p.x2 = !(dgrad && hk == 1 && !g.bnr_x2);
      p.grid_x = (unsigned)(ntiles < slots ? ntiles : slots);
      p.rows = (int)p.grid_x;
      return p;
    }
    if (variant == 6) {
      p.err = (int)hipErrorInvalidValue;
      return p;
    }
    variant = dgrad ? (g.Ncols <= 64 ? 5 : 2) : 2;
    if (!dgrad || g.st == 1) variant = conv_default_variant(g, variant);
  }
  p.variant = variant;
  if (variant == 0 || (dgrad && g.st > 2)) {
    p.family = kConvReg;
    p.BM = conv_small_m(g, false) ? 64 : 128;
    p.BN = conv_bn(g);
    p.WM = p.WN = 2;
    p.rows = (int)((M + p.BM - 1) / p.BM);
    p.grid_x = (unsigned)(nx * p.rows);
    return p;
  }
  p.family = kConvPipe;
  p.par = dgrad && g.st == 2;
  conv_pipe_tile_of(g, dgrad, p.par, variant, [&](auto t) {
    using T = decltype(t);
    p.BM = T::BM; p.BN = T::BN; p.WM = T::WM; p.WN = T::WN; p.STAGES = T::STAGES; p.KS = T::KS; p.KG = T::KG;
    return 0;
  });
  if (p.KG > 1 && !g.vec) p.err = (int)hipErrorInvalidValue;
  const size_t ring = (size_t)p.KG * p.STAGES * (p.BM + p.BN) * p.KS * sizeof(bf16_t);
  const size_t kgred = p.KG > 1 ? (size_t)p.KG * p.BM * (p.BN + 4) * sizeof(float) : 0;
  p.lds = ring > kgred ? ring : kgred;
  p.x2 = !(dgrad && !p.par && !g.bnr_x2);
  p.fast = p.par ? (g.IC % p.KS == 0 && (!g.X2 || g.K2 % p.KS == 0) && ((g.R + 1) / 2) * ((g.S + 1) / 2) <= 32)
                 : (g.IC % p.KS == 0 && g.R * g.S <= 32 && (!dgrad || g.st == 1));
  const long nbn = (g.Ncols + p.BN - 1) / p.BN;
  if (!p.par) {
    p.rows = (int)((M + p.BM - 1) / p.BM);
    p.grid_x = (unsigned)(p.rows * nbn);
    return p;
  }
  p.grid_y = 4;
  for (int cls = 0; cls < 4; ++cls) {
    const int ph = cls >> 1, pw = cls & 1;
    const long Mc = (long)g.N * ((g.OH - ph + 1) >> 1) * ((g.OW - pw + 1) >> 1);
    p.rows += (int)((Mc + p.BM - 1) / p.BM);
    if (cls == 0) p.grid_x = (unsigned)((Mc + p.BM - 1) / p.BM * nbn);
  }
  return p;
}

template <bool DGRAD>
int launch_conv_plan(ConvGeom& g, const ConvPlan& p, hipStream_t st) {
  if (p.err != (int)hipSuccess) return p.err;
  if (p.family == kConvHalo) return launch_conv_halo<DGRAD>(g, p, st);
  if (p.family == kConvReg) return launch_conv<DGRAD>(g, p, st);
  if constexpr (DGRAD)
    if (p.par)
      return conv_pipe_tile<true, true>(g, p.variant,
                                        [&](auto t) { return launch_conv_pipe_t<true, true, decltype(t)>(g, p, st); });
  return conv_pipe_tile<DGRAD, false>(g, p.variant,
                                      [&](auto t) { return launch_conv_pipe_t<DGRAD, false, decltype(t)>(g, p, st); });
}

int conv_plan_rows(const ConvGeom& g, bool dgrad, int variant) {
  const ConvPlan p = conv_plan(g, dgrad, variant);
  if (p.family == kConvHalo || (variant == -1 && p.family == kConvPipe)) return p.rows;
  return (int)(((long)g.N * g.OH * g.OW + 63) / 64 + (dgrad ? 4 : 0));
}

ConvGeom fwd_geom(int N, int H, int W, int C, int K, int R, int S, int stride, int pad, const void* x,
                  const void* w_packed, void* y, float* stats) {
  ConvGeom g{};
  g.N = N; g.IH = H; g.IW = W; g.IC = C;
  g.OH = (H + 2 * pad - R) / stride + 1; g.OW = (W + 2 * pad - S) / stride + 1;
  g.R = R; g.S = S; g.st = stride; g.pad = pad;
  g.Ncols = K; g.Kred = R * S * C;
  g.X = (const bf16_t*)x; g.Wt = (const bf16_t*)w_packed; g.Y = (bf16_t*)y; g.ldy = K; g.stats = stats;
  g.vec = conv_vec_ok(g);
  return g;
}

ConvGeom dgrad_geom(int N, int H, int W, int C, int K, int R, int S, int stride, int pad, const void* dy,
                    const void* wt_packed, const void* ds_dy) {
  ConvGeom g{};
  g.N = N; g.OH = H; g.OW = W;
  g.IH = (H + 2 * pad - R) / stride + 1; g.IW = (W + 2 * pad - S) / stride + 1; g.IC = K;
  g.R = R; g.S = S; g.st = stride; g.pad = pad;
  g.Ncols = C; g.Kred = R * S * K;
  g.X = (const bf16_t*)dy; g.Wt = (const bf16_t*)wt_packed; g.ldy = C; g.stats = nullptr;
  g.X2 = (const bf16_t*)ds_dy;
  g.vec = conv_vec_ok(g);
  return g;
}

}

MER_API int mer_conv_fwd(int N, int H, int W, int C, int K, int R, int S, int stride, int pad, const void* x,
                         const void* w_packed, void* y, float* stats, void* stream) {
  return mer_conv_fwd_ex(N, H, W, C, K, R, S, stride, pad, x, w_packed, y, stats, -1, stream);
}

MER_API int mer_conv_fwd_rows(int N, int H, int W, int C, int K, int R, int S, int stride, int pad, const void* x,
                              const void* w_packed, int variant) {
  if (N <= 0 || C % 8 || variant < -1 || variant > 7) return -(int)hipErrorInvalidValue;
  return conv_plan_rows(fwd_geom(N, H, W, C, K, R, S, stride, pad, x, w_packed, nullptr, nullptr), false, variant);
}

MER_API int mer_conv_dgrad_rows(int N, int H, int W, int C, int K, int R, int S, int stride, int pad, const void* dy,
                                const void* wt_packed, const void* ds_dy, int variant) {
  if (N <= 0 || K % 8 || C % 8 || variant < -1 || variant > 7) return -(int)hipErrorInvalidValue;
  return conv_plan_rows(dgrad_geom(N, H, W, C, K, R, S, stride, pad, dy, wt_packed, ds_dy), true, variant);
}

MER_API int mer_conv_fwd_ex(int N, int H, int W, int C, int K, int R, int S, int stride, int pad, const void* x,
                            const void* w_packed, void* y, float* stats, int variant, void* stream) {
  if (C % 8 || variant < -1 || variant > 7) return (int)hipErrorInvalidValue;
  ConvGeom g = fwd_geom(N, H, W, C, K, R, S, stride, pad, x, w_packed, y, stats);
  return launch_conv_plan<false>(g, conv_plan(g, false, variant), (hipStream_t)stream);
}

MER_API int mer_conv_dgrad(int N, int H, int W, int C, int K, int R, int S, int stride, int pad, const void* dy,
                           const void* wt_packed, void* dx, const void* residual, const void* residual_mask,
                           void* stream) {
  return mer_conv_dgrad_ex(N, H, W, C, K, R, S, stride, pad, dy, wt_packed, dx, residual, residual_mask, -1, stream);
}

MER_API int mer_conv_dgrad_ex(int N, int H, int W, int C, int K, int R, int S, int stride, int pad, const void* dy,
                              const void* wt_packed, void* dx, const void* residual, const void* residual_mask,
                              int variant, void* stream) {
  return mer_conv_dgrad_bnr(N, H, W, C, K, R, S, stride, pad, dy, wt_packed, dx, residual, residual_mask, nullptr,
                            nullptr, nullptr, nullptr, nullptr, nullptr, nullptr, variant, stream);
}

MER_API int mer_conv_dgrad_bnr(int N, int H, int W, int C, int K, int R, int S, int stride, int pad, const void* dy,
                               const void* wt_packed, void* dx, const void* residual, const void* residual_mask,
                               const void* bn_mask, const void* bn_x, const float* bn_ms, float* bn_red,
                               const void* bn_x2, const float* bn_ms2, float* bn_red2, int variant, void* stream) {
  return mer_conv_dgrad_ds(N, H, W, C, K, R, S, stride, pad, dy, wt_packed, dx, residual, residual_mask, bn_mask, bn_x,
                           bn_ms, bn_red, bn_x2, bn_ms2, bn_red2, nullptr, nullptr, 0, variant, stream);
}

MER_API int mer_conv_dgrad_ds(int N, int H, int W, int C, int K, int R, int S, int stride, int pad, const void* dy,
                              const void* wt_packed, void* dx, const void* residual, const void* residual_mask,
                              const void* bn_mask, const void* bn_x, const float* bn_ms, float* bn_red,
                              const void* bn_x2, const float* bn_ms2, float* bn_red2, const void* ds_dy,
                              const void* ds_wt_packed, int ds_K, int variant, void* stream) {
  if (K % 8 || C % 8 || variant < -1 || variant > 7) return (int)hipErrorInvalidValue;
  if (ds_dy && (stride != 2 || R != 3 || S != 3 || pad != 1 || !ds_wt_packed || ds_K <= 0 || ds_K % 64 || K % 64 ||
                variant == 0))
    return (int)hipErrorInvalidValue;
  if (bn_red && (!bn_mask || !bn_x || !bn_ms || (bn_x2 && (!bn_ms2 || !bn_red2)))) return (int)hipErrorInvalidValue;
  if (bn_red && (variant == 0 || stride > 2)) return (int)hipErrorInvalidValue;
  ConvGeom g = dgrad_geom(N, H, W, C, K, R, S, stride, pad, dy, wt_packed, ds_dy);
  g.Y = (bf16_t*)dx;
  g.R_ = (const bf16_t*)residual; g.Rmask = (const bf16_t*)residual_mask;
  g.bnr_mask = (const bf16_t*)bn_mask; g.bnr_x = (const bf16_t*)bn_x; g.bnr_ms = bn_ms; g.bnr_red = bn_red;
  g.bnr_x2 = (const bf16_t*)bn_x2; g.bnr_ms2 = bn_ms2; g.bnr_red2 = bn_red2;
  g.Wt2 = (const bf16_t*)ds_wt_packed; g.K2 = ds_dy ? ds_K : 0;
  return launch_conv_plan<true>(g, conv_plan(g, true, variant), (hipStream_t)stream);
}
```

### multimodalemotionrecognition_amd/csrc/conv_common.h

```cpp
#pragma once
#include <type_traits>

#include "common.h"
#include "mer.h"

typedef __attribute__((ext_vector_type(4))) uint32_t u32x4;
typedef __attribute__((ext_vector_type(4))) short s16x4;

#ifdef MER_CONV_TIMING
#define MER_CT_BUFFER(name, words) \
  static __device__ long long name##_buf[words]; \
  MER_API int name##_reset() { \
    static long long zeros[words]; \
    return (int)hipMemcpyToSymbol(HIP_SYMBOL(name##_buf), zeros, sizeof(zeros), 0, hipMemcpyHostToDevice); \
  } \
  MER_API int name##_read(long long* host) { \
    return (int)hipMemcpyFromSymbol(host, HIP_SYMBOL(name##_buf), sizeof(long long) * (words), 0, \
                                    hipMemcpyDeviceToHost); \
  }
#define MER_CT_MODE_WORD(name) \
  static __device__ int name##_v; \
  MER_API int name(int mode) { \
    return (int)hipMemcpyToSymbol(HIP_SYMBOL(name##_v), &mode, sizeof(int), 0, hipMemcpyHostToDevice); \
  }
#define CT_AT(buf, k) \
  do { \
    if (threadIdx.x == 0 && blockIdx.x < 512 && (k) < 64) buf[blockIdx.x * 64 + (k)] = wall_clock64(); \
  } while (0)
#define CTP_AT(buf, k) \
  do { \
    const unsigned b_ = blockIdx.y * gridDim.x + blockIdx.x; \
    if (threadIdx.x == 0 && b_ < 4096) buf[b_ * 8 + (k)] = wall_clock64(); \
  } while (0)
#else
#define MER_CT_BUFFER(name, words)
#define MER_CT_MODE_WORD(name)
#define CT_AT(buf, k) \
  do { \
  } while (0)
#define CTP_AT(buf, k) \
  do { \
  } while (0)
#endif

namespace {

constexpr int CBK = 64;

struct ConvGeom {
  int N, OH, OW;
  int IH, IW, IC;
  int R, S, st, pad;
  int Ncols;
  int Kred;
  const bf16_t* X;
  const bf16_t* Wt;
  bf16_t* Y;
  long ldy;
  float* stats;
  const bf16_t* R_;
  const bf16_t* Rmask;
  const bf16_t* bnr_mask;
  const bf16_t* bnr_x;
  const float* bnr_ms;
  float* bnr_red;
  const bf16_t* bnr_x2;
  const float* bnr_ms2;
  float* bnr_red2;
  int vec;
  const bf16_t* X2;
  const bf16_t* Wt2;
  int K2;
};

__host__ __device__ inline bool conv_vec_ok(const ConvGeom& g) {
  const uintptr_t a = (uintptr_t)g.Y | (uintptr_t)g.R_ | (uintptr_t)g.Rmask | (uintptr_t)g.bnr_mask |
                      (uintptr_t)g.bnr_x | (uintptr_t)g.bnr_x2 | (uintptr_t)g.stats | (uintptr_t)g.bnr_red |
                      (uintptr_t)g.bnr_red2;
  return g.Ncols % 8 == 0 && g.ldy % 8 == 0 && (a & 15) == 0;
}

static __device__ __attribute__((aligned(16))) uint32_t mer_conv_zero16[4] = {0u, 0u, 0u, 0u};

int cu_count() {
  static const int n = [] {
    int dev = 0, v = 0;
    if (hipGetDevice(&dev) != hipSuccess || hipDeviceGetAttribute(&v, hipDeviceAttributeMultiprocessorCount, dev) !=
                                                hipSuccess || v <= 0)
      return 256;
    return v;
  }();
  return n;
}

}
```

### multimodalemotionrecognition_amd/kernels.py

```python
from __future__ import annotations

import os

import torch

from ._lib import LIB, MerKernelError

F32, BF16 = 0, 1
ACT = {"none": 0, "relu": 1, "gelu": 2}


def stream_ptr() -> int:
    return torch.cuda.current_stream().cuda_stream


class KernelProbe:

    def __init__(self, name: str, key: tuple, units: float):
        self.name, self.key, self.units = name, tuple(key), units
        self.pairs = []
        self.active = False

    def matches(self, name, key):
        return self.active and name == self.name and tuple(key) == self.key
# ... 294 lines not shown
    return float(drop_p), rng_ptr(rng) if drop_p > 0 else 0, int(site), _ptr(skip), int(skip_bit)


def gemm_bf16(a, w, out, *, M=None, K=None, rows=None, bias=None, residual=None, act="none", variant=-1,
              drop_p=0.0, rng=None, site=0, skip=None, skip_bit=0):
    N = w.shape[0]
    if rows is None:
        M, K = a.shape
        rows = (M, a.stride(0), 0)
    if w.dtype != torch.bfloat16 or a.dtype != torch.bfloat16 or w.shape[1] != K or w.stride(1) != 1:
        raise ValueError("gemm_bf16 expects bf16 A and W[N,K]")
    if out.shape[-1] != N or out.numel() != M * N:
        raise ValueError(f"gemm_bf16 out shape {tuple(out.shape)} != ({M},{N})")
    _aligned16(a, w)
    ldc = N if out.dim() < 2 else out.stride(-2)
    ldr = 0 if residual is None else residual.stride(-2)
    if drop_p > 0 or skip is not None:
        _launch("gemm_bf16", (M, N, K), "mer_gemm_bf16_tr", M, N, K, a.data_ptr(), rows[2], rows[1], rows[0],
                w.data_ptr(), w.stride(0), out.data_ptr(), _dt(out), ldc, _ptr(bias), _ptr(residual), ldr, ACT[act],
                *_train_args(drop_p, rng, site, skip, skip_bit), int(variant), stream_ptr())
        return out
    _launch("gemm_bf16", (M, N, K), "mer_gemm_bf16_ex", M, N, K, a.data_ptr(), rows[2], rows[1], rows[0], w.data_ptr(),
            w.stride(0), out.data_ptr(), _dt(out), ldc, _ptr(bias), _ptr(residual), ldr, ACT[act], int(variant),
            stream_ptr())
    return out


def posconv_gemm_bf16(x, wp, out, B, L, C, groups, taps, pad, bias, residual, act="gelu", variant=-1):
    LIB("mer_posconv_gemm_bf16", B, L, C, groups, taps, pad, x.data_ptr(), x.stride(-2), wp.data_ptr(), out.data_ptr(),
        _dt(out), out.stride(-2), _ptr(bias), _ptr(residual), 0 if residual is None else residual.stride(-2),
        ACT[act], int(variant), stream_ptr())


def wavlm_conv0_gn_gelu(wav, w0, gamma, beta, out, eps=1e-5):
    B, S = wav.shape
    Lout = out.shape[1]
    if tuple(out.shape) != (B, (S - 10) // 5 + 1, 512) or out.dtype != torch.bfloat16:
        raise ValueError(f"wavlm_conv0_gn_gelu out {tuple(out.shape)}")
    ws = torch.empty(B * ((Lout + 127) // 128 + 1) * 1024 + 16384, device=wav.device, dtype=torch.float32)
    LIB("mer_wavlm_conv0_gn_gelu", B, S, Lout, wav.data_ptr(), w0.data_ptr(), gamma.data_ptr(), beta.data_ptr(),
        float(eps), ws.data_ptr(), out.data_ptr(), stream_ptr())


def layernorm(x2d, gamma, beta, y2d, eps=1e-5, drop_p=0.0, rng=None, site=0, skip=None, skip_bit=0):
    rows, d = x2d.shape
    if drop_p > 0 or skip is not None:
        LIB("mer_layernorm_tr", rows, d, x2d.data_ptr(), _dt(x2d), x2d.stride(0), gamma.data_ptr(), beta.data_ptr(),
            float(eps), y2d.data_ptr(), _dt(y2d), y2d.stride(0), *_train_args(drop_p, rng, site, skip, skip_bit),
            stream_ptr())
        return
    LIB("mer_layernorm", rows, d, x2d.data_ptr(), _dt(x2d), x2d.stride(0), gamma.data_ptr(), beta.data_ptr(),
        float(eps), y2d.data_ptr(), _dt(y2d), y2d.stride(0), stream_ptr())


def wavlm_attention(qkv, x, gate_w, gate_b, gate_const, rel_emb, bucket, out, B, L, H, scale, drop_p=0.0, rng=None,
                    site=0, skip=None, skip_bit=0):
    if drop_p > 0 or skip is not None:
        LIB("mer_wavlm_attention_tr", B, L, H, qkv.data_ptr(), qkv.stride(0), x.data_ptr(), x.stride(0),
            gate_w.data_ptr(), gate_b.data_ptr(), gate_const.data_ptr(), rel_emb.data_ptr(), _ptr(bucket),
            out.data_ptr(), out.stride(0), float(scale), *_train_args(drop_p, rng, site, skip, skip_bit), stream_ptr())
        return
    LIB("mer_wavlm_attention", B, L, H, qkv.data_ptr(), qkv.stride(0), x.data_ptr(), x.stride(0), gate_w.data_ptr(),
        gate_b.data_ptr(), gate_const.data_ptr(), rel_emb.data_ptr(), _ptr(bucket), out.data_ptr(),
        out.stride(0), float(scale), stream_ptr())


def wavlm_time_mask(h, B, L, embed, mask_prob, mask_len, min_masks, rng, site, mask_out=None):
    D = h.shape[-1]
    if h.dtype != torch.bfloat16 or h.numel() != B * L * D or embed.numel() != D:
        raise ValueError("wavlm_time_mask shapes")
    if mask_len > L:
        raise ValueError(f"`mask_length` has to be smaller than `sequence_length`, but got `mask_length`: {mask_len} "
                         f"and `sequence_length`: {L}`")
    if mask_out is not None and (mask_out.dtype != torch.uint8 or mask_out.numel() != B * L):
        raise ValueError("mask_out must be uint8 [B, L]")
    LIB("mer_wavlm_time_mask", B, L, D, h.data_ptr(), h.stride(-2), embed.detach().contiguous().data_ptr(),
        float(mask_prob), int(mask_len), int(min_masks), rng_ptr(rng), int(site), _ptr(mask_out), stream_ptr())


def bf16_convert(x, y):
    if x.dtype != torch.bfloat16 or not x.is_contiguous() or not y.is_contiguous() or x.numel() != y.numel():
        raise ValueError("bf16_convert: contiguous bf16 source of the same size")
    LIB("mer_bf16_convert", x.numel(), x.data_ptr(), y.data_ptr(), _dt(y), stream_ptr())
    return y


def permute3_bf16(src, shape3, strides3, dst, scale=None):
    n0, n1, n2 = shape3
    LIB("mer_permute3_bf16", n0, n1, n2, src.data_ptr(), strides3[0], strides3[1], strides3[2], _ptr(scale),
        dst.data_ptr(), stream_ptr())


def weightnorm_scale(v, g, scale):
    n01 = v.shape[0] * v.shape[1]
    LIB("mer_weightnorm_scale", n01, v.shape[2], v.data_ptr(), g.data_ptr(), scale.data_ptr(), stream_ptr())


def cast_bf16(x, y):
    LIB("mer_cast_bf16", x.numel(), x.data_ptr(), y.data_ptr(), stream_ptr())


BN_STAT_PARTS = 64


def bn_stat_rows(M: int) -> int:
    return (M + 63) // 64 + 64


def bn_red_rows(M: int) -> int:
    return (M + 63) // 64 + 4 + 64


BN_RED_WS_ROWS = 576


def bn_stats_buffer(C, device, M=None):
    rows = BN_STAT_PARTS if M is None else bn_stat_rows(M)
    return torch.zeros(rows, C, 2, device=device, dtype=torch.float32)


def conv_fwd(x, wp, y, stats, R, S, stride, pad, variant=-1):
    N, H, W, C = x.shape
    Kc = y.shape[-1]
    Ho, Wo = (H + 2 * pad - R) // stride + 1, (W + 2 * pad - S) // stride + 1
    if tuple(y.shape) != (N, Ho, Wo, Kc) or tuple(wp.shape) != (Kc, R * S * C):
        raise ValueError(f"conv_fwd shapes x{tuple(x.shape)} w{tuple(wp.shape)} y{tuple(y.shape)}")
    if stats is not None and (stats.numel() != bn_stat_rows(N * Ho * Wo) * Kc * 2 or not stats.is_contiguous()):
        raise ValueError("conv_fwd stats must be a contiguous zeroed float[bn_stat_rows(M)][K][2] buffer")
    _launch("conv_fwd", (N, H, W, C, Kc, R, stride), "mer_conv_fwd_ex", N, H, W, C, Kc, R, S, stride, pad, x.data_ptr(),
            wp.data_ptr(), y.data_ptr(), _ptr(stats), int(variant), stream_ptr())
    if stats is not None:
        return _partial_rows("mer_conv_fwd_rows", N, H, W, C, Kc, R, S, stride, pad, x.data_ptr(), wp.data_ptr(),
                             int(variant))
    return None


_ROWS_CACHE = {}
PARTIAL_ROWS = True


def _partial_rows(fn, *args):
    if not PARTIAL_ROWS:
        return None
    key = (fn,) + tuple(a % 16 == 0 if isinstance(a, int) and a > 1 << 20 else a for a in args)
    r = _ROWS_CACHE.get(key)
    if r is None:
        r = int(LIB.call_int(fn, *args))
        if r <= 0:
            raise MerKernelError(f"{fn}{args[:9]} failed: {r}")
        _ROWS_CACHE[key] = r
    return r


def conv_dgrad(dy, wt, dx, R, S, stride, pad, residual=None, mask=None, variant=-1, bnr=None, ds=None):
    N, H, W, C = dx.shape
    Kc = dy.shape[-1]
    Ho, Wo = (H + 2 * pad - R) // stride + 1, (W + 2 * pad - S) // stride + 1
    if tuple(dy.shape) != (N, Ho, Wo, Kc) or tuple(wt.shape) != (C, R * S * Kc):
        raise ValueError(f"conv_dgrad shapes dy{tuple(dy.shape)} wt{tuple(wt.shape)} dx{tuple(dx.shape)}")
    b = list(bnr) + [None] * (7 - len(bnr)) if bnr is not None else [None] * 7
    for t in (b[0], b[1], b[4]):
        if t is not None and tuple(t.shape) != tuple(dx.shape):
            raise ValueError("conv_dgrad bnr tensors must match dx")
    for t in (b[3], b[6]):
        if t is not None and t.numel() != bn_red_rows(N * H * W) * C * 2:
            raise ValueError("conv_dgrad bnr red buffers must be zeroed [bn_red_rows(N*H*W), C, 2]")
    if ds is not None:
        ddy, dwt = ds
        Kd = ddy.shape[-1]
        if tuple(ddy.shape) != (N, Ho, Wo, Kd) or tuple(dwt.shape) != (C, Kd) or stride != 2 or R != 3 or pad != 1:
            raise ValueError("conv_dgrad ds: a 1x1 / stride-2 downsample gradient beside a 3x3 / stride-2 / pad-1 conv")
        _launch("conv_dgrad", (N, H, W, C, Kc, R, stride), "mer_conv_dgrad_ds", N, H, W, C, Kc, R, S, stride, pad,
                dy.data_ptr(), wt.data_ptr(), dx.data_ptr(), _ptr(residual), _ptr(mask), *[_ptr(t) for t in b],
                ddy.data_ptr(), dwt.data_ptr(), Kd, int(variant), stream_ptr())
    else:
        _launch("conv_dgrad", (N, H, W, C, Kc, R, stride), "mer_conv_dgrad_bnr", N, H, W, C, Kc, R, S, stride, pad,
                dy.data_ptr(), wt.data_ptr(), dx.data_ptr(), _ptr(residual), _ptr(mask), *[_ptr(t) for t in b],
                int(variant), stream_ptr())
    if bnr is None:
        return None
    return _partial_rows("mer_conv_dgrad_rows", N, H, W, C, Kc, R, S, stride, pad, dy.data_ptr(), wt.data_ptr(),
                         ds[0].data_ptr() if ds is not None else 0, int(variant))


def partials_sum(parts_buf, out, rows=None):
    P, C, _ = parts_buf.shape
    if P <= 64:
        raise ValueError("partials_sum expects a bn_red_rows(M) buffer (data rows + 64 scratch rows)")
    if rows is None:
        rows = P - 64
    if not 0 < rows <= P - 64:
        raise ValueError("partials_sum rows out of range")
    LIB("mer_partials_sum", C, int(rows), parts_buf.data_ptr(), out.data_ptr(), stream_ptr())
    return out


_WGRAD_WGS = 768
WGRAD_VARIANT = 8
_WGRAD_STRIP_KB = {9: 64, 10: 32}
_WGRAD_STRIP_WGS = 256


def wgrad_strip_split_count(N: int, H: int, splits: int) -> int:
    rows = N * (H + 1)
    per = -(-rows // max(1, int(splits)))
    return -(-rows // per)


def _wgrad_min_pix(out_elems, tiles):
    return 256 if out_elems <= 65536 else (512 if tiles >= 96 else 1024)


def wgrad_split_count(P: int, splits: int) -> int:
    splits = max(1, int(splits))
    pps = (-(-P // splits) + 63) // 64 * 64
    return -(-P // pps)


class WgradFolds:

    MAX = 32

    def __init__(self):
        self.rows, self.keep = [], []

    def add(self, ws, dw, Kc, C, creal, RS, splits, map_=None):
        self.rows.append([ws.data_ptr(), dw.data_ptr(), _ptr(map_), Kc, C, creal, RS, splits])
        self.keep += [ws, dw, map_]

    def flush(self):
        import numpy as np
        for i in range(0, len(self.rows), self.MAX):
            tab = np.ascontiguousarray(np.array(self.rows[i:i + self.MAX], dtype=np.int64))
            _launch("wgrad_fold_batch", (len(tab),), "mer_wgrad_fold_batch", len(tab), tab.ctypes.data, stream_ptr())
        self.rows, self.keep = [], []


def conv_wgrad(x, dy, dw, R, S, stride, pad, creal=None, variant=-1, splits=None, defer=None, dw_map=None):
    N, H, W, C = x.shape
    Kc = dy.shape[-1]
    Ho, Wo = (H + 2 * pad - R) // stride + 1, (W + 2 * pad - S) // stride + 1
    creal = C if creal is None else creal
    if dw_map is not None:
        if defer is None or dw_map.dtype != torch.int32 or dw_map.numel() != R * S * C or not dw.is_contiguous():
            raise ValueError("conv_wgrad dw_map: deferred fold, int32 [R*S*C], contiguous dw")
        if dw.shape[0] != Kc or dw.dtype != torch.float32:
            raise ValueError("conv_wgrad shapes")
    elif tuple(dy.shape) != (N, Ho, Wo, Kc) or tuple(dw.shape) != (Kc, creal, R, S) or dw.dtype != torch.float32:
        raise ValueError("conv_wgrad shapes")
    if tuple(dy.shape) != (N, Ho, Wo, Kc):
        raise ValueError("conv_wgrad shapes")
    P = N * Ho * Wo
    tiles = ((Kc + 127) // 128) * ((R * S * C + 127) // 128)
    if variant == -1:
        variant = WGRAD_VARIANT if (Kc > 64 and stride == 1 and R * S > 1) else 4
    strip = variant in _WGRAD_STRIP_KB
    kg = 2 if variant == 8 else 1
    if strip:
        if splits is None:
            stiles = max(1, (C // 64) * (Kc // _WGRAD_STRIP_KB[variant]))
            splits = max(1, min(_WGRAD_STRIP_WGS // stiles, N * (H + 1) * (W + 1) // 1024))
        eff = wgrad_strip_split_count(N, H, splits)
    else:
        if splits is None:
            splits = int(max(1, min(-(-_WGRAD_WGS // (kg * tiles)),
                                    P // (kg * _wgrad_min_pix(Kc * R * S * C, tiles)))))
        eff = wgrad_split_count(P, splits)
    ws = torch.empty(splits * Kc * R * S * C, device=x.device, dtype=torch.float32)
    if defer is not None:
        _launch("conv_wgrad", (N, H, W, C, Kc, R, stride), "mer_conv_wgrad_partials", N, H, W, C, Kc, R, S, stride,
                pad, x.data_ptr(), dy.data_ptr(), int(splits), ws.data_ptr(), int(variant), stream_ptr())
        defer.add(ws, dw, Kc, C, dw.numel() // Kc if dw_map is not None else creal, R * S, eff, dw_map)
        return
    _launch("conv_wgrad", (N, H, W, C, Kc, R, stride), "mer_conv_wgrad_ex", N, H, W, C, creal, Kc, R, S, stride, pad,
            x.data_ptr(), dy.data_ptr(), dw.data_ptr(), int(splits), ws.data_ptr(), int(variant), stream_ptr())


def pack_input_s2d(x, y):
    N, C, H, W = x.shape
    if tuple(y.shape) != (N, H // 2 + 3, W // 2 + 3, 16) or y.dtype != torch.bfloat16 or not y.is_contiguous():
        raise ValueError("pack_input_s2d shapes")
    if x.dtype != torch.float32 or not x.is_contiguous():
        raise ValueError("pack_input_s2d reads contiguous fp32 NCHW frames")
    LIB("mer_pack_input_s2d", N, C, H, W, x.data_ptr(), y.data_ptr(), stream_ptr())


def pack_input_nhwc(x, y):
    N, C, H, W = x.shape
    LIB("mer_pack_input_nhwc", N, C, H, W, y.shape[-1], x.data_ptr(), y.data_ptr(), stream_ptr())


def pack_conv_weight(w, out, cp, transpose):
    Kc, C, R, S = w.shape
    LIB("mer_pack_conv_weight", Kc, C, R, S, cp, int(transpose), w.data_ptr(), out.data_ptr(), stream_ptr())


def pack_conv_weights(desc, blocks, flat=True):
    if desc.dtype != torch.int64 or desc.dim() != 2 or desc.shape[1] != 9 or not desc.is_cuda:
        raise ValueError("pack descriptor table must be a device int64 [n, 9] tensor")
    name = "mer_pack_conv_weights_flat" if flat else "mer_pack_conv_weights"
    LIB(name, desc.shape[0], desc.data_ptr(), int(blocks), stream_ptr())


def bn_finalize(stats, M, eps, momentum, ms, rmean=None, rvar=None, nbt=None, rows=None):
    C = ms.shape[0]
    if stats is not None and (stats.numel() != bn_stat_rows(int(M)) * C * 2 or not stats.is_contiguous()):
        raise ValueError("bn_finalize stats must be the conv_fwd float[bn_stat_rows(M)][C][2] buffer")
    if rows is None:
        rows = bn_stat_rows(int(M)) - 64
    LIB("mer_bn_finalize_rows", C, int(M), int(rows), _ptr(stats), float(eps), float(momentum), ms.data_ptr(),
        _ptr(rmean), _ptr(rvar), _ptr(nbt), stream_ptr())


def bn_finalize_pair(a, b, eps, momentum):
    args = []
    for stats, M, ms, rmean, rvar, nbt, rows in (a, b):
        C = ms.shape[0]
        if stats is None or stats.numel() != bn_stat_rows(int(M)) * C * 2 or not stats.is_contiguous():
            raise ValueError("bn_finalize_pair stats must be conv_fwd float[bn_stat_rows(M)][C][2] buffers")
        rows = bn_stat_rows(int(M)) - 64 if rows is None else rows
        args += [C, int(M), int(rows), stats.data_ptr(), ms.data_ptr(), _ptr(rmean), _ptr(rvar), _ptr(nbt)]
    LIB("mer_bn_finalize_rows2", *args, float(eps), float(momentum), stream_ptr())


def partials_sum_pair(buf_a, out_a, buf_b, out_b, rows=None):
    P, C, _ = buf_a.shape
    if tuple(buf_b.shape) != (P, C, 2) or P <= 64:
        raise ValueError("partials_sum_pair expects two bn_red_rows(M) buffers of one shape")
    rows = P - 64 if rows is None else rows
    if not 0 < rows <= P - 64:
        raise ValueError("partials_sum_pair rows out of range")
    LIB("mer_partials_sum2", C, int(rows), buf_a.data_ptr(), out_a.data_ptr(), buf_b.data_ptr(), out_b.data_ptr(),
        stream_ptr())
    return out_a, out_b


def bn_apply(x, ms, gamma, beta, y, relu, res=None, ms2=None, gamma2=None, beta2=None):
    C = x.shape[-1]
    M = x.numel() // C
    LIB("mer_bn_apply", M, C, x.data_ptr(), ms.data_ptr(), gamma.data_ptr(), beta.data_ptr(), _ptr(res), _ptr(ms2),
        _ptr(gamma2), _ptr(beta2), int(relu), y.data_ptr(), stream_ptr())


def bn_bwd_reduce(dy, mask, x, ms, red, workspace=None):
    C = x.shape[-1]
    if workspace is None:
        workspace = torch.empty(BN_RED_WS_ROWS * C * 2, device=x.device, dtype=torch.float32)
    if workspace.numel() < BN_RED_WS_ROWS * C * 2:
        raise ValueError("bn_bwd_reduce workspace too small")
    LIB("mer_bn_bwd_reduce", x.numel() // C, C, dy.data_ptr(), _ptr(mask), x.data_ptr(), ms.data_ptr(),
        red.data_ptr(), workspace.data_ptr(), stream_ptr())


def bn_bwd_apply(dy, mask, x, ms, gamma, red, dx, dgamma, dbeta, batch_stats=True):
    C = x.shape[-1]
    LIB("mer_bn_bwd_apply", x.numel() // C, C, dy.data_ptr(), _ptr(mask), x.data_ptr(), ms.data_ptr(),
        gamma.data_ptr(), red.data_ptr(), int(batch_stats), dx.data_ptr(), _ptr(dgamma), _ptr(dbeta), stream_ptr())


def bn_bwd_apply2(dy, mask, x, ms, gamma, red, dx, dgamma, dbeta, x2, ms2, gamma2, red2, dx2, dgamma2, dbeta2,
                  batch_stats=True):
    C = x.shape[-1]
    for t in (dy, mask, x2, dx, dx2):
        if tuple(t.shape) != tuple(x.shape):
            raise ValueError("bn_bwd_apply2 tensors must share one shape")
    LIB("mer_bn_bwd_apply2", x.numel() // C, C, dy.data_ptr(), mask.data_ptr(), x.data_ptr(), ms.data_ptr(),
        gamma.data_ptr(), red.data_ptr(), x2.data_ptr(), ms2.data_ptr(), gamma2.data_ptr(), red2.data_ptr(),
        int(batch_stats), dx.data_ptr(), dx2.data_ptr(), _ptr(dgamma), _ptr(dbeta), _ptr(dgamma2), _ptr(dbeta2),
        stream_ptr())


def maxpool_fwd(x, y, arg):
    N, H, W, C = x.shape
    LIB("mer_maxpool_fwd", N, H, W, C, x.data_ptr(), y.data_ptr(), arg.data_ptr(), stream_ptr())


def stem_bnrelu_maxpool(x, ms, gamma, beta, y, arg):
    N, H, W, C = x.shape
    LIB("mer_stem_bnrelu_maxpool_fwd", N, H, W, C, x.data_ptr(), ms.data_ptr(), gamma.data_ptr(), beta.data_ptr(),
        y.data_ptr(), arg.data_ptr(), stream_ptr())


def stem_pool_bn_bwd(dy, arg, x, ms, gamma, beta, red, dx, dgamma, dbeta, batch_stats=True, workspace=None):
    N, H, W, C = x.shape
    if workspace is None:
        workspace = torch.empty(BN_RED_WS_ROWS * C * 2, device=x.device, dtype=torch.float32)
    if workspace.numel() < BN_RED_WS_ROWS * C * 2:
        raise ValueError("stem_pool_bn_bwd workspace too small")
    LIB("mer_stem_pool_bn_bwd", N, H, W, C, dy.data_ptr(), arg.data_ptr(), x.data_ptr(), ms.data_ptr(),
        gamma.data_ptr(), beta.data_ptr(), red.data_ptr(), int(batch_stats), dx.data_ptr(), _ptr(dgamma),
        _ptr(dbeta), workspace.data_ptr(), stream_ptr())


def maxpool_bwd(dy, arg, dx):
    N, H, W, C = dx.shape
    LIB("mer_maxpool_bwd", N, H, W, C, dy.data_ptr(), arg.data_ptr(), dx.data_ptr(), stream_ptr())


def avgpool_fwd(x, y):
    N, H, W, C = x.shape
    LIB("mer_avgpool_fwd", N, H * W, C, x.data_ptr(), y.data_ptr(), stream_ptr())


def avgpool_bwd(dy, dx):
    N, H, W, C = dx.shape
    LIB("mer_avgpool_bwd", N, H * W, C, dy.data_ptr(), dx.data_ptr(), stream_ptr())


def softmax_avg_fwd(za, zv, out, pa, pv):
    B, C = za.shape
    LIB("mer_softmax_avg_fwd", B, C, za.data_ptr(), zv.data_ptr(), out.data_ptr(), pa.data_ptr(), pv.data_ptr(),
        stream_ptr())


def softmax_avg_bwd(pa, pv, dout, da, dv):
    B, C = pa.shape
    LIB("mer_softmax_avg_bwd", B, C, pa.data_ptr(), pv.data_ptr(), dout.data_ptr(), da.data_ptr(), dv.data_ptr(),
        stream_ptr())


QP_PARTIAL = 2 * 512


def quant_params(x, partial, qparams, mode):
    _check_dev(x, partial, qparams)
    if not x.is_contiguous() or x.data_ptr() % 16:
        raise ValueError("quant_params needs a contiguous 16-byte aligned tensor")
    LIB("mer_quant_params", x.numel(), x.data_ptr(), _dt(x), partial.data_ptr(), int(mode), qparams.data_ptr(),
        stream_ptr())


def quantize_weight_s8(w, qparams, qw, colsum):
    N, K = w.shape
    if qw.shape[0] != N or qw.shape[1] < K or qw.shape[1] % 16 or qw.dtype != torch.int8:
        raise ValueError("qw must be int8 [N, ldq>=K], ldq % 16 == 0")
    LIB("mer_quantize_weight_s8", N, K, w.data_ptr(), w.stride(0), qparams.data_ptr(), qw.data_ptr(), qw.stride(0),
        colsum.data_ptr(), stream_ptr())


def gemm_i8dyn(x2d, x_qparams, qw, w_qparams, colsum, bias, out, act="none"):
    _check_dev(x2d, qw, out)
    M, K = x2d.shape
    N = qw.shape[0]
    if x2d.stride(1) != 1 or x2d.stride(0) % 8 or K % 16 or out.shape != (M, N) or x2d.data_ptr() % 16:
        raise ValueError(f"gemm_i8dyn: bad operands x{tuple(x2d.shape)} qw{tuple(qw.shape)} out{tuple(out.shape)}")
    _launch("gemm_i8dyn", (M, N, K), "mer_gemm_i8dyn", M, N, K, x2d.data_ptr(), _dt(x2d), x2d.stride(0), x_qparams.data_ptr(),
            qw.data_ptr(), qw.stride(0), w_qparams.data_ptr(), colsum.data_ptr(), _ptr(bias), ACT[act], out.data_ptr(),
            out.stride(0), stream_ptr())
    return out


def _ptr0(t):
    return 0 if t is None else t.data_ptr()


def fold_rows(part, parts, n, ldp, out, offset=0):
    if out.dtype != torch.float32 or not out.is_contiguous() or out.numel() != n:
        raise ValueError("fold_rows: out must be contiguous fp32 of n elements")
    if offset + (parts - 1) * ldp + n > part.numel():
        raise ValueError("fold_rows: partial rows out of range")
    ws = _workspace(64 * n, out.device) if parts > 64 else None
    LIB("mer_fold_rows", int(parts), int(n), part.data_ptr() + 4 * offset, int(ldp), out.data_ptr(), _ptr0(ws),
        stream_ptr())


def ln_bwd(dy_a, x, gamma, eps, dy_b=None, dy_c=None, dx32=None, dx16=None):
    rows, d = x.shape
    for t in (dy_a, dy_b, dy_c, dx32):
        if t is not None and (t.dtype != torch.float32 or tuple(t.shape) != (rows, d) or not t.is_contiguous()):
            raise ValueError("ln_bwd: fp32 [rows, d] contiguous operands expected")
    if dx16 is not None and (dx16.dtype != torch.bfloat16 or tuple(dx16.shape) != (rows, d)):
        raise ValueError("ln_bwd: dx16 must be bf16 [rows, d]")
    if x.dtype != torch.float32 or not x.is_contiguous() or d % 256 or d > 1024:
        raise ValueError("ln_bwd: x must be contiguous fp32 with d % 256 == 0, d <= 1024")
    part = _workspace(((rows + 15) // 16) * 3 * d, x.device)
    LIB("mer_ln_bwd", rows, d, dy_a.data_ptr(), _ptr0(dy_b), _ptr0(dy_c), x.data_ptr(), gamma.data_ptr(), float(eps),
        _ptr0(dx32), _ptr0(dx16), part.data_ptr(), stream_ptr())
    return part


def ln_bwd_fold(part, rows, d, dgamma=None, dbeta=None, dbias=None):
    parts = (rows + 15) // 16
    for i, out in enumerate((dgamma, dbeta, dbias)):
        if out is not None:
            fold_rows(part, parts, d, 3 * d, out, offset=i * d)


def colsum_into(x2d, out, col0=0, ncols=None):
    rows, cols = x2d.shape
    part = _workspace(((rows + 63) // 64) * cols, x2d.device)
    LIB("mer_colpart", rows, cols, x2d.data_ptr(), _dt(x2d), x2d.stride(0), part.data_ptr(), stream_ptr())
    ncols = cols - col0 if ncols is None else ncols
    fold_rows(part, (rows + 63) // 64, ncols, cols, out, offset=col0)


def gelu_bf16(z, f):
    if z.dtype != torch.bfloat16 or f.dtype != torch.bfloat16 or z.numel() != f.numel() or z.numel() % 8:
        raise ValueError("gelu_bf16: bf16 operands of equal size (multiple of 8)")
    LIB("mer_gelu_bf16", z.numel(), z.data_ptr(), f.data_ptr(), stream_ptr())


def gelu_bwd(df, z, dz, dbias):
    rows, cols = z.shape
    if df.dtype != torch.float32 or tuple(df.shape) != (rows, cols) or dz.dtype != torch.bfloat16:
        raise ValueError("gelu_bwd shapes")
    part = _workspace(((rows + 63) // 64) * cols, z.device)
    LIB("mer_gelu_bwd", rows, cols, df.data_ptr(), z.data_ptr(), dz.data_ptr(), part.data_ptr(), stream_ptr())
    fold_rows(part, (rows + 63) // 64, cols, cols, dbias)


def linear_wgrad(x, dy, dw, col0=0):
    M, Kin = x.shape
    N = dw.shape[0]
    if (x.dtype != torch.bfloat16 or dy.dtype != torch.bfloat16 or dw.dtype != torch.float32 or not x.is_contiguous()
            or tuple(dw.shape) != (N, Kin) or dy.shape[0] != M or dy.shape[1] < col0 + N or dy.stride(1) != 1
            or Kin % 8 or N % 8 or col0 % 8 or dy.stride(0) % 8):
        raise ValueError("linear_wgrad shapes")
    tiles = ((N + 127) // 128) * ((Kin + 127) // 128)
    splits = int(max(1, min(-(-512 // tiles), M // 512)))
    ws = _workspace(splits * N * Kin, x.device)
    LIB("mer_linear_wgrad", M, N, Kin, x.data_ptr(), dy.data_ptr() + 2 * col0, dy.stride(0), dw.data_ptr(), splits,
        ws.data_ptr(), stream_ptr())


def _attn_bwd_kp(L):
    nt = -(-L // 16)
    return 16 * (4 if nt <= 4 else 8 if nt <= 8 else 10 if nt <= 10 else 12)


def wavlm_attention_bwd(qkv, x, dout, gate_w, gate_b, gate_const, tbl, B, L, H, scale, dqkv, dx_gate=None,
                        drop_p=0.0, rng=None, site=0):
    M = B * L
    if L > 192 or tuple(qkv.shape) != (M, 3 * H * 64) or tuple(dqkv.shape) != (M, 3 * H * 64) or dout.shape[0] != M:
        raise ValueError("wavlm_attention_bwd shapes")
    if qkv.dtype != torch.bfloat16 or dout.dtype != torch.float32 or dqkv.dtype != torch.bfloat16:
        raise ValueError("wavlm_attention_bwd expects bf16 qkv / dqkv and fp32 dout")
    if tuple(tbl.shape) != (H, 2 * L - 1) or tbl.dtype != torch.float32:
        raise ValueError("wavlm_attention_bwd: bias table [H, 2L-1] fp32")
    kp = _attn_bwd_kp(L)
    scratch = torch.empty(B * H * kp * (3 * kp + 64), device=qkv.device, dtype=torch.bfloat16)
    nrb = (L + 63) // 64
    gpart = _workspace(B * H * nrb * (8 * 64 + 8 + H), qkv.device)
    tr = _train_args(drop_p, rng, site, None, 0)[:3]
    LIB("mer_wavlm_attention_bwd_tr", B, L, H, qkv.data_ptr(), qkv.stride(0), x.data_ptr(), x.stride(0),
        dout.data_ptr(), dout.stride(0), gate_w.data_ptr(), gate_b.data_ptr(), gate_const.data_ptr(), tbl.data_ptr(),
        float(scale), scratch.data_ptr(), dqkv.data_ptr(), dqkv.stride(0), _ptr0(dx_gate),
        dx_gate.stride(0) if dx_gate is not None else 0, gpart.data_ptr(), *tr, stream_ptr())
    return gpart, B * H * nrb


def dropout_rows(x, drop_p, rng, site, y32=None, y16=None):
    rows, cols = x.shape
    for y in (y32, y16):
        if y is not None and tuple(y.shape) != (rows, cols):
            raise ValueError("dropout_rows output shape")
    if (y32 is not None and y32.dtype != torch.float32) or (y16 is not None and y16.dtype != torch.bfloat16):
        raise ValueError("dropout_rows: y32 fp32, y16 bf16")
    tr = _train_args(drop_p, rng, site, None, 0)[:3]
    LIB("mer_dropout_rows", rows, cols, x.data_ptr(), _dt(x), x.stride(0), _ptr0(y32),
# ... 274 lines not shown
```

### multimodalemotionrecognition_amd/video.py

```python
from __future__ import annotations

import os
import warnings
from typing import List

import torch
from torch import nn

from . import graphs as G
from . import kernels as K
from .nn_ops import hip_linear
from .optim import weight_version
from .temporal import TemporalPooler

S2D_CH = 16


class BasicBlock(nn.Module):
    expansion = 1

    def __init__(self, inplanes: int, planes: int, stride: int = 1, downsample: nn.Module = None):
        super().__init__()
        self.conv1 = nn.Conv2d(inplanes, planes, 3, stride, 1, bias=False)
        self.bn1 = nn.BatchNorm2d(planes)
# ... 315 lines not shown
    Ho, Wo = (H + 2 * pad - R) // stride + 1, (W + 2 * pad - S) // stride + 1
    y = torch.empty(N, Ho, Wo, Kc, device=x.device, dtype=torch.bfloat16)
    stats = None
    if training:
        M = N * Ho * Wo
        stats = arena.take(Kc, M=M) if arena is not None else K.bn_stats_buffer(Kc, x.device, M)
    rows = K.conv_fwd(x, trunk.packed(conv, C, False), y, stats, R, S, stride, pad)
    if defer:
        return y, stats, rows
    return y, _bn_forward(bn, y, stats, training, rows)


def _bn_forward_pair(bns, ys, stats, rows):
    recs, out = [], []
    for bn, y, st, r in zip(bns, ys, stats, rows):
        C = y.shape[-1]
        ms = torch.empty(C, 2, device=y.device, dtype=torch.float32)
        if (0.1 if bn.momentum is None else bn.momentum) != (0.1 if bns[0].momentum is None else bns[0].momentum) \
                or bn.eps != bns[0].eps:
            raise ValueError("paired BatchNorm finalize needs one eps / momentum")
        recs.append((st, y.numel() // C, ms, bn.running_mean, bn.running_var, bn.num_batches_tracked, r))
        out.append(ms)
    K.bn_finalize_pair(recs[0], recs[1], bns[0].eps, 0.1 if bns[0].momentum is None else bns[0].momentum)
    return out


@torch.no_grad()
def block_forward(trunk, blk: BasicBlock, x: torch.Tensor, training: bool, arena=None):
    s = blk.stride
    bc1, bms1 = _conv_bn(trunk, blk.conv1, blk.bn1, x, s, 1, training, arena)
    ba1 = torch.empty_like(bc1)
    K.bn_apply(bc1, bms1, blk.bn1.weight, blk.bn1.bias, ba1, relu=True)
    dbn = blk.downsample[1] if blk.downsample is not None else None
    paired = dbn is not None and training and BN_FIN_PAIR
    if paired:
        bc2, st2, r2 = _conv_bn(trunk, blk.conv2, blk.bn2, ba1, 1, 1, training, arena, defer=True)
        cd, std, rd = _conv_bn(trunk, blk.downsample[0], dbn, x, s, 0, training, arena, defer=True)
        bms2, msd = _bn_forward_pair((blk.bn2, dbn), (bc2, cd), (st2, std), (r2, rd))
    else:
        bc2, bms2 = _conv_bn(trunk, blk.conv2, blk.bn2, ba1, 1, 1, training, arena)
    out = torch.empty_like(bc2)
    if blk.downsample is not None:
        if not paired:
            cd, msd = _conv_bn(trunk, blk.downsample[0], blk.downsample[1], x, s, 0, training, arena)
        K.bn_apply(bc2, bms2, blk.bn2.weight, blk.bn2.bias, out, relu=True, res=cd, ms2=msd, gamma2=dbn.weight,
                   beta2=dbn.bias)
    else:
        cd = msd = None
        K.bn_apply(bc2, bms2, blk.bn2.weight, blk.bn2.bias, out, relu=True, res=x)
    return out, (x, bc1, bms1, ba1, bc2, bms2, cd, msd, out)


class _ForcePack:

    def __init__(self, trunk, on):
        self.trunk, self.on = trunk, on

    def __enter__(self):
        self.prev = self.trunk._force_pack
        self.trunk._force_pack = self.on or self.prev

    def __exit__(self, *exc):
        self.trunk._force_pack = self.prev


@torch.no_grad()
def trunk_forward(trunk: ResNet18Trunk, video: torch.Tensor, training: bool, force_pack: bool = False,
                  s2d: torch.Tensor = None):
    with _ForcePack(trunk, force_pack):
        return _trunk_forward(trunk, video, training, s2d)


def s2d_input(video: torch.Tensor, out: torch.Tensor = None) -> torch.Tensor:
    N, C, H, W = video.shape
    video = video.float().contiguous()
    if out is None:
        out = torch.empty(N, H // 2 + 3, W // 2 + 3, S2D_CH, device=video.device, dtype=torch.bfloat16)
    K.pack_input_s2d(video, out)
    return out


def _trunk_forward(trunk: ResNet18Trunk, video: torch.Tensor, training: bool, s2d: torch.Tensor = None):
    trunk.pack_all(transpose=False)
    N, C, H, W = video.shape
    dev = video.device
    bf = torch.bfloat16
    conv1, bn1 = trunk[0], trunk[1]
    _check_stem(conv1, C, H, W)
    if s2d is None:
        x0 = s2d_input(video)
    else:
        if tuple(s2d.shape) != (N, H // 2 + 3, W // 2 + 3, S2D_CH) or s2d.dtype != bf:
            raise ValueError(f"packed frames {tuple(s2d.shape)} do not match video {tuple(video.shape)}")
        x0 = s2d
    arena = _StatsArena(trunk, dev, floats=_fwd_stat_floats(trunk, N, H, W), zero=not K.PARTIAL_ROWS) \
        if training else None
    c1, ms1 = _conv_bn(trunk, conv1, bn1, x0, 1, 0, training, arena, rs=(4, 4))
    Hp, Wp = (c1.shape[1] - 1) // 2 + 1, (c1.shape[2] - 1) // 2 + 1
    p1 = torch.empty(N, Hp, Wp, c1.shape[-1], device=dev, dtype=bf)
    arg = torch.empty(N, Hp, Wp, c1.shape[-1], device=dev, dtype=torch.uint8)
    K.stem_bnrelu_maxpool(c1, ms1, bn1.weight, bn1.bias, p1, arg)
    saved = {"stem": (x0, c1, ms1, arg), "blocks": []}
    x = p1
    for blk in _blocks(trunk):
        x, sv = block_forward(trunk, blk, x, training, arena)
        saved["blocks"].append(sv)
    feats = torch.empty(N, x.shape[-1], device=dev, dtype=torch.float32)
    K.avgpool_fwd(x, feats)
    saved["final"] = x
    return feats, saved


def _grad(param, grads):
    from .fusion import grad_buffer

    if not param.requires_grad:
        return None
    g = grads.get(id(param))
    if g is None:
        g = grad_buffer(param)
        grads[id(param)] = g
    return g


def _bn_bwd(g, mask, x, ms, bn, red, grads, training):
    dx = torch.empty_like(x)
    K.bn_bwd_apply(g, mask, x, ms, bn.weight, red, dx, _grad(bn.weight, grads), _grad(bn.bias, grads), training)
    return dx


def _block_bwd_floats(sv) -> int:
    xin, bc1, _, ba1, bc2, _, _, _, out = sv
    C1, C2, Cin = bc1.shape[-1], bc2.shape[-1], xin.shape[-1]
    return 2 * (K.bn_red_rows(ba1.numel() // C1) * C1 + 2 * K.BN_RED_WS_ROWS * C2 + C2 * 2
                + 2 * K.bn_red_rows(xin.numel() // Cin) * Cin)


def _bnr_target(blk_sv, blk, arena):
    xin, bc1, bms1, ba1, bc2, bms2, cd, msd, out = blk_sv
    C2 = bc2.shape[-1]
    rows = K.bn_red_rows(out.numel() // C2)
    red2 = arena.take(C2, parts=rows)
    if cd is None:
        return (out, bc2, bms2, red2), (red2, None)
    redd = arena.take(C2, parts=rows)
    return (out, bc2, bms2, red2, cd, msd, redd), (red2, redd)


WGRAD_DEFER = True
BN_BWD_PAIR = True
BN_FIN_PAIR = True
FOLD_EVERY = 2
FUSED_DS_DGRAD = True


class _WgradLane:

    def __init__(self, device):
        self.folds = K.WgradFolds() if WGRAD_DEFER else None

    def run(self, fn, *reads, block=None):
        fn()

    def join(self):
        if self.folds is not None:
            self.folds.flush()


@torch.no_grad()
def block_backward(trunk, blk: BasicBlock, sv, dx: torch.Tensor, grads, training: bool = True, pre=None,
                   prev=None, arena=None, lane=None, bidx=None):
    dev = dx.device
    xin, bc1, bms1, ba1, bc2, bms2, cd, msd, out = sv
    if arena is None:
        arena = _StatsArena(trunk, dev, floats=_block_bwd_floats(sv))
    own_lane = lane is None
    if own_lane:
        lane = _WgradLane(dev)
    g_out = dx
    s = blk.stride
    C2 = bc2.shape[-1]
    if pre is not None:
        if cd is not None and BN_FIN_PAIR:
            red2, redd = K.partials_sum_pair(pre[0], torch.empty(C2, 2, device=dev, dtype=torch.float32), pre[1],
                                             torch.empty(C2, 2, device=dev, dtype=torch.float32), pre[2])
        else:
            red2 = K.partials_sum(pre[0], torch.empty(C2, 2, device=dev, dtype=torch.float32), pre[2])
            redd = K.partials_sum(pre[1], torch.empty(C2, 2, device=dev, dtype=torch.float32), pre[2]) \
                if cd is not None else None
    else:
        red2 = arena.take(C2, parts=1)
        K.bn_bwd_reduce(g_out, out, bc2, bms2, red2, arena.take(C2, parts=K.BN_RED_WS_ROWS))
        redd = None
        if cd is not None:
            redd = arena.take(C2, parts=1)
            K.bn_bwd_reduce(g_out, out, cd, msd, redd, arena.take(C2, parts=K.BN_RED_WS_ROWS))
    if cd is not None and BN_BWD_PAIR:
        dc2, dcd = torch.empty_like(bc2), torch.empty_like(cd)
        bd = blk.downsample[1]
        K.bn_bwd_apply2(g_out, out, bc2, bms2, blk.bn2.weight, red2, dc2, _grad(blk.bn2.weight, grads),
                        _grad(blk.bn2.bias, grads), cd, msd, bd.weight, redd, dcd, _grad(bd.weight, grads),
                        _grad(bd.bias, grads), training)
    else:
        dc2 = _bn_bwd(g_out, out, bc2, bms2, blk.bn2, red2, grads, training)
        dcd = _bn_bwd(g_out, out, cd, msd, blk.downsample[1], redd, grads, training) if cd is not None else None
    w2 = _grad(blk.conv2.weight, grads)
    if w2 is not None:
        lane.run(lambda: K.conv_wgrad(ba1, dc2, w2, 3, 3, 1, 1, defer=lane.folds), ba1, dc2, w2, block=bidx)
    da1 = torch.empty_like(ba1)
    C1 = bc1.shape[-1]
    red1p = arena.take(C1, parts=K.bn_red_rows(ba1.numel() // C1))
    rows1 = K.conv_dgrad(dc2, trunk.packed(blk.conv2, C2, True), da1, 3, 3, 1, 1, bnr=(ba1, bc1, bms1, red1p))
    red1 = K.partials_sum(red1p, torch.empty(C1, 2, device=dev, dtype=torch.float32), rows1)
    dc1 = _bn_bwd(da1, ba1, bc1, bms1, blk.bn1, red1, grads, training)
    w1 = _grad(blk.conv1.weight, grads)
    if w1 is not None:
        lane.run(lambda: K.conv_wgrad(xin, dc1, w1, 3, 3, s, 1, defer=lane.folds), xin, dc1, w1, block=bidx)
    dxin = torch.empty_like(xin)
    Cin = xin.shape[-1]
    bnr, nxt = _bnr_target(prev[0], prev[1], arena) if prev is not None else (None, None)
    if cd is not None:
        wd = _grad(blk.downsample[0].weight, grads)
        if wd is not None:
            lane.run(lambda: K.conv_wgrad(xin, dcd, wd, 1, 1, s, 0, defer=lane.folds), xin, dcd, wd, block=bidx)
        if FUSED_DS_DGRAD and s == 2:
            rows = K.conv_dgrad(dc1, trunk.packed(blk.conv1, Cin, True), dxin, 3, 3, s, 1, bnr=bnr,
                                ds=(dcd, trunk.packed(blk.downsample[0], Cin, True)))
        else:
            dxd = torch.empty_like(xin)
            K.conv_dgrad(dcd, trunk.packed(blk.downsample[0], Cin, True), dxd, 1, 1, s, 0)
            rows = K.conv_dgrad(dc1, trunk.packed(blk.conv1, Cin, True), dxin, 3, 3, s, 1, residual=dxd, bnr=bnr)
    else:
        rows = K.conv_dgrad(dc1, trunk.packed(blk.conv1, Cin, True), dxin, 3, 3, s, 1, residual=g_out, mask=out,
                            bnr=bnr)
    if own_lane:
        lane.join()
    return dxin, (nxt + (rows,) if nxt is not None else None)


@torch.no_grad()
def trunk_backward(trunk: ResNet18Trunk, saved, dfeat: torch.Tensor, training: bool = True, force_pack: bool = False,
                   hook=None):
    split = SPLIT_BLOCK if hook is not None else 0
    state = trunk_backward_start(trunk, saved, dfeat, training, split, force_pack=force_pack)
    if hook is not None:
        hook(trunk.split_params(split))
    return trunk_backward_finish(trunk, saved, state, training, force_pack=force_pack)


@torch.no_grad()
def trunk_backward_start(trunk, saved, dfeat, training, split, force_pack=False):
    with _ForcePack(trunk, force_pack):
        trunk.pack_all(transpose=True)
        dev = dfeat.device
        x = saved["final"]
        dx = torch.empty_like(x)
        K.avgpool_bwd(dfeat, dx)
        svs = saved["blocks"]
        arena = _StatsArena(trunk, dev, floats=sum(_block_bwd_floats(sv) for sv in svs) + 2 * K.BN_RED_WS_ROWS * 64 * 2)
        state = dict(dx=dx, pre=None, grads={}, arena=arena, i=len(svs) - 1, lane=_WgradLane(dev))
        _backward_blocks(trunk, saved, state, max(split, trunk.backward_stop(), 0), training)
        state["lane"].join()
        return state


def _backward_blocks(trunk, saved, state, lo, training):
    blocks, svs = _blocks(trunk), saved["blocks"]
    while state["i"] >= lo:
        i = state["i"]
        prev = (svs[i - 1], blocks[i - 1]) if i > 0 else None
        state["dx"], state["pre"] = block_backward(trunk, blocks[i], svs[i], state["dx"], state["grads"], training,
                                                   pre=state["pre"], prev=prev, arena=state["arena"],
                                                   lane=state["lane"], bidx=i)
        if FOLD_EVERY and i % FOLD_EVERY == 0 and i > 0:
            state["lane"].join()
        state["i"] = i - 1


@torch.no_grad()
def trunk_backward_finish(trunk, saved, state, training, force_pack=False):
    with _ForcePack(trunk, force_pack):
        stop = trunk.backward_stop()
        _backward_blocks(trunk, saved, state, max(stop, 0), training)
        grads, arena, dx = state["grads"], state["arena"], state["dx"]
        if stop >= 0:
            state["lane"].join()
            return grads
        dev = dx.device
        x0, c1, ms1, arg = saved["stem"]
        bn1 = trunk[1]
        red = arena.take(c1.shape[-1], parts=1)
        dc1 = torch.empty_like(c1)
        K.stem_pool_bn_bwd(dx, arg, c1, ms1, bn1.weight, bn1.bias, red, dc1, _grad(bn1.weight, grads),
                           _grad(bn1.bias, grads), training, workspace=arena.take(c1.shape[-1], parts=K.BN_RED_WS_ROWS))
        w = _grad(trunk[0].weight, grads)
        if w is not None:
            Kc, Cin, R, S = trunk[0].weight.shape
            Ro, So = (R + 2) // 2, (S + 2) // 2
            folds = state["lane"].folds
            if folds is not None:
                K.conv_wgrad(x0, dc1, w, Ro, So, 1, 0, defer=folds, dw_map=trunk.stem_wgrad_table(dev, True))
            else:
                ws2d = torch.empty(Kc, S2D_CH, Ro, So, device=dev, dtype=torch.float32)
                ws2d.zero_()
                K.conv_wgrad(x0, dc1, ws2d, Ro, So, 1, 0)
                idx = trunk.stem_wgrad_table(dev, False)
                w.add_(ws2d.view(Kc, -1).index_select(1, idx).view_as(w))
        state["lane"].join()
        return grads


class VideoNet(nn.Module):

    def __init__(self, num_classes: int, pretrained: bool = True, temporal_pooling: str = "mean",
                 temporal_num_heads: int = 4, temporal_num_layers: int = 1, temporal_dropout: float = 0.1) -> None:
        super().__init__()
        if pretrained:
            warnings.warn("ImageNet weights are a network fetch in the reference (video.py:21); building the "
                          "resnet18 trunk from random init offline")
        self.backbone = ResNet18Trunk()
        self.embedding_dim = 512
        self.temporal_pool = TemporalPooler(self.embedding_dim, temporal_pooling, temporal_num_heads,
                                            temporal_num_layers, temporal_dropout)
        self.classifier = nn.Linear(self.embedding_dim, num_classes)

    def encode(self, x: torch.Tensor) -> torch.Tensor:
        b, t, c, h, w = x.shape
        feat = self.backbone(x.view(b * t, c, h, w)).view(b, t, self.embedding_dim)
        return self.temporal_pool(feat)

    def forward(self, x: torch.Tensor) -> torch.Tensor:
        return hip_linear(self.encode(x), self.classifier)
```

Measured before the change: 223.4 steps/s.

## Carry ReLU mask into stored dgrad outputs so BN backward skips mask reads

Applies the ReLU mask once, when each gradient is written (in the dgrad epilogue and in avgpool backward), so the stored gradient is already masked. Downstream BN reduce/apply and the residual-add path can then pass a null mask and skip reading the mask tensor again. The cost is an extra mask read and select inside the dgrad epilogue, plus a separate re-walk pass over the output for the large PAR tile configuration, which may add register pressure or extra memory traffic there.

```diff
diff --git a/include/mer.h b/include/mer.h
--- a/include/mer.h
+++ b/include/mer.h
@@ -208,6 +208,11 @@
                       const void* bn_mask, const void* bn_x, const float* bn_ms, float* bn_red, const void* bn_x2,
                       const float* bn_ms2, float* bn_red2, const void* ds_dy, const void* ds_wt_packed, int ds_K,
                       int variant, void* stream);
+int mer_conv_dgrad_carry(int N, int H, int W, int C, int K, int R, int S, int stride, int pad, const void* dy,
+                         const void* wt_packed, void* dx, const void* residual, const void* residual_mask,
+                         const void* bn_mask, const void* bn_x, const float* bn_ms, float* bn_red, const void* bn_x2,
+                         const float* bn_ms2, float* bn_red2, const void* ds_dy, const void* ds_wt_packed, int ds_K,
+                         int store_masked, int variant, void* stream);
 
 int mer_conv_fwd_rows(int N, int H, int W, int C, int K, int R, int S, int stride, int pad, const void* x,
                       const void* w_packed, int variant);
@@ -266,6 +271,7 @@
 
 int mer_avgpool_fwd(int N, int HW, int C, const void* x, float* y, void* stream);
 int mer_avgpool_bwd(int N, int HW, int C, const float* dy, void* dx, void* stream);
+int mer_avgpool_bwd_masked(int N, int HW, int C, const float* dy, const void* mask, void* dx, void* stream);
 
 
 int mer_quant_params(long n, const void* x, int x_dtype, float* partial, int mode, float* qparams, void* stream);
diff --git a/multimodalemotionrecognition_amd/csrc/bn_pool.hip b/multimodalemotionrecognition_amd/csrc/bn_pool.hip
--- a/multimodalemotionrecognition_amd/csrc/bn_pool.hip
+++ b/multimodalemotionrecognition_amd/csrc/bn_pool.hip
@@ -611,9 +611,10 @@
   for (int j = 0; j < 6; ++j)
 #pragma unroll
     for (int i = 0; i < 8; ++i) k[j][i] = coef[j][c0 + i];
+  const u32x4 one16 = {0x3f803f80u, 0x3f803f80u, 0x3f803f80u, 0x3f803f80u};
   for (long e = tid0; e < nvec; e += stride) {
     const u32x4 gv = *reinterpret_cast<const u32x4*>(dy + e * 8);
-    const u32x4 mv = *reinterpret_cast<const u32x4*>(mask + e * 8);
+    const u32x4 mv = mask ? *reinterpret_cast<const u32x4*>(mask + e * 8) : one16;
     const u32x4 xv = *reinterpret_cast<const u32x4*>(x + e * 8);
     const u32x4 x2v = *reinterpret_cast<const u32x4*>(x2 + e * 8);
     const bf16_t* gh = reinterpret_cast<const bf16_t*>(&gv);
@@ -637,7 +638,7 @@
                               const float* gamma, const float* red, const void* x2, const float* ms2,
                               const float* gamma2, const float* red2, int batch_stats, void* dx, void* dx2,
                               float* dgamma, float* dbeta, float* dgamma2, float* dbeta2, void* stream) {
-  if (C % 8 || C > 512 || 256 % (C / 8) || !mask || !x2 || !dx2 || dx == dy || dx2 == dy)
+  if (C % 8 || C > 512 || 256 % (C / 8) || !x2 || !dx2 || dx == dy || dx2 == dy)
     return (int)hipErrorInvalidValue;
   const long nvec = M * C / 8;
   const int grid = bn_stream_grid(nvec);
@@ -840,11 +841,14 @@
   for (int p = 0; p < HW; ++p) s += bf2f(x[((long)n * HW + p) * C + c]);
   y[(long)n * C + c] = s / HW;
 }
-__global__ void avgpool_bwd_kernel(int N, int HW, int C, const float* __restrict__ dy, bf16_t* __restrict__ dx) {
+__global__ void avgpool_bwd_kernel(int N, int HW, int C, const float* __restrict__ dy,
+                                   const bf16_t* __restrict__ mask, bf16_t* __restrict__ dx) {
   const int n = blockIdx.y;
   for (int e = blockIdx.x * blockDim.x + threadIdx.x; e < HW * C; e += gridDim.x * blockDim.x) {
     const int c = e % C;
-    dx[(long)n * HW * C + e] = f2bf(dy[(long)n * C + c] / HW);
+    const long at = (long)n * HW * C + e;
+    const bool live = !mask || bf2f(mask[at]) > 0.f;
+    dx[at] = live ? f2bf(dy[(long)n * C + c] / HW) : (bf16_t)0;
   }
 }
 MER_API int mer_avgpool_fwd(int N, int HW, int C, const void* x, float* y, void* stream) {
@@ -853,7 +857,11 @@
   MER_LAUNCH_CHECK();
 }
 MER_API int mer_avgpool_bwd(int N, int HW, int C, const float* dy, void* dx, void* stream) {
+  return mer_avgpool_bwd_masked(N, HW, C, dy, nullptr, dx, stream);
+}
+MER_API int mer_avgpool_bwd_masked(int N, int HW, int C, const float* dy, const void* mask, void* dx, void* stream) {
   dim3 grid((HW * C + 255) / 256, N);
-  hipLaunchKernelGGL(avgpool_bwd_kernel, grid, dim3(256), 0, (hipStream_t)stream, N, HW, C, dy, (bf16_t*)dx);
-  MER_LAUNCH_CHECK();
-}
+  hipLaunchKernelGGL(avgpool_bwd_kernel, grid, dim3(256), 0, (hipStream_t)stream, N, HW, C, dy, (const bf16_t*)mask,
+                     (bf16_t*)dx);
+  MER_LAUNCH_CHECK();
+}
diff --git a/multimodalemotionrecognition_amd/csrc/conv.hip b/multimodalemotionrecognition_amd/csrc/conv.hip
--- a/multimodalemotionrecognition_amd/csrc/conv.hip
+++ b/multimodalemotionrecognition_amd/csrc/conv.hip
@@ -347,7 +347,7 @@
 }
 
 template <bool DGRAD, int FM, int FN, int WM, int WN, int WAVE_FLOATS, class OutRow, class Pre = EpiNone,
-          bool DEFER = false, bool X2 = true, class AccT = EpiNoAcc>
+          bool DEFER = false, bool X2 = true, class AccT = EpiNoAcc, bool YMWALK = false>
 __device__ __forceinline__ void conv_epilogue_vec(const ConvGeom& g, f32x4 (&acc)[FM][FN], float* smemf, int w,
                                                   int lane, int m0, int n0, int M, long red_row_id, long stat_row,
                                                   OutRow out_row, const Pre* pre = nullptr, int ct_slot = -1,
@@ -367,6 +367,7 @@
   const bool cok = colv < g.Ncols;
   const bool do_bnr = DGRAD && g.bnr_red != nullptr;
   const bool has_x2 = X2 && do_bnr && g.bnr_x2 != nullptr;
+  const bool ymask = do_bnr && g.y_masked != 0;
   float mu[8], rs[8], mu2[8], rs2[8];
   float sA[8], sB[8], sC[8];
   constexpr int NPS = DEFER ? E::NP : 1;
@@ -396,6 +397,8 @@
     }
     sA[e] = sB[e] = sC[e] = 0.f;
   }
+  auto passes = [&](auto ym_tag) {
+  constexpr bool YM = decltype(ym_tag)::value;
 #pragma unroll
   for (int i0 = 0; i0 < FM; i0 += GI) {
 #pragma unroll
@@ -420,7 +423,21 @@
         float v[8] = {lo[0], lo[1], lo[2], lo[3], hi[0], hi[1], hi[2], hi[3]};
         const long e0 = out_row(row) * g.ldy + colv;
         const int q = (i0 / GI) * E::PPG + rr / RPP;
-        if (DGRAD && g.R_) {
+        u32x4 bmv = {0u, 0u, 0u, 0u};
+        if constexpr (YM) {
+          if constexpr (PREF) bmv = pre->bm[q];
+          else bmv = *reinterpret_cast<const u32x4*>(g.bnr_mask + e0);
+        }
+        if constexpr (YM) {
+          if (g.R_) {
+            u32x4 rv;
+            if constexpr (PREF) rv = pre->r[q];
+            else rv = *reinterpret_cast<const u32x4*>(g.R_ + e0);
+            const bf16_t* rh = reinterpret_cast<const bf16_t*>(&rv);
+#pragma unroll
+            for (int e = 0; e < 8; ++e) v[e] += bf2f(rh[e]);
+          }
+        } else if (DGRAD && g.R_) {
           u32x4 rv, mv;
           if constexpr (PREF) {
             rv = pre->r[q];
@@ -442,6 +459,14 @@
           oh[e] = f2bf(v[e]);
           v[e] = bf2f(oh[e]);
         }
+        if constexpr (YM) {
+          const bf16_t* mh = reinterpret_cast<const bf16_t*>(&bmv);
+#pragma unroll
+          for (int e = 0; e < 8; ++e) {
+            v[e] = bf2f(mh[e]) > 0.f ? v[e] : 0.f;
+            oh[e] = f2bf(v[e]);
+          }
+        }
         if constexpr (DEFER) {
           pend[q] = ov;
           pend_at[q] = e0;
@@ -449,23 +474,23 @@
         } else {
           *reinterpret_cast<u32x4*>(g.Y + e0) = ov;
         }
-        if (do_bnr) {
-          u32x4 mv, xv, x2v;
+        if (YM || do_bnr) {
+          u32x4 xv, x2v;
           if constexpr (PREF) {
-            mv = pre->bm[q];
+            if constexpr (!YM) bmv = pre->bm[q];
             xv = pre->x[q];
             x2v = pre->x2[q];
           } else {
-            mv = *reinterpret_cast<const u32x4*>(g.bnr_mask + e0);
+            if constexpr (!YM) bmv = *reinterpret_cast<const u32x4*>(g.bnr_mask + e0);
             xv = *reinterpret_cast<const u32x4*>(g.bnr_x + e0);
             x2v = has_x2 ? *reinterpret_cast<const u32x4*>(g.bnr_x2 + e0) : u32x4{0u, 0u, 0u, 0u};
           }
-          const bf16_t* mh = reinterpret_cast<const bf16_t*>(&mv);
+          const bf16_t* mh = reinterpret_cast<const bf16_t*>(&bmv);
           const bf16_t* xh = reinterpret_cast<const bf16_t*>(&xv);
           const bf16_t* x2h = reinterpret_cast<const bf16_t*>(&x2v);
 #pragma unroll
           for (int e = 0; e < 8; ++e) {
-            const float gv = bf2f(mh[e]) > 0.f ? v[e] : 0.f;
+            const float gv = (YM || bf2f(mh[e]) > 0.f) ? v[e] : 0.f;
             sA[e] += gv;
             sB[e] += gv * (bf2f(xh[e]) - mu[e]) * rs[e];
             if (has_x2) sC[e] += gv * (bf2f(x2h[e]) - mu2[e]) * rs2[e];
@@ -477,6 +502,35 @@
     __builtin_amdgcn_wave_barrier();
     __builtin_amdgcn_fence(__ATOMIC_ACQUIRE, "wavefront");
   }
+  };
+  if (DGRAD && !YMWALK && ymask) {
+    if constexpr (DGRAD && !YMWALK) passes(std::true_type{});
+  } else {
+    passes(std::false_type{});
+  }
+  if constexpr (DGRAD && YMWALK && !DEFER) {
+    if (ymask) {
+#pragma unroll
+      for (int i0 = 0; i0 < FM; i0 += GI) {
+        const int nrows = (FM - i0 < GI ? FM - i0 : GI) * 16;
+#pragma unroll
+        for (int rr = 0; rr < GI * 16; rr += RPP) {
+          const int rl = rr + lr;
+          const int row = m0 + wr * TM + i0 * 16 + rl;
+          if (rl < nrows && row < M && cok) {
+            const long e0 = out_row(row) * g.ldy + colv;
+            u32x4 yv = *reinterpret_cast<const u32x4*>(g.Y + e0);
+            const u32x4 bmv = *reinterpret_cast<const u32x4*>(g.bnr_mask + e0);
+            bf16_t* yh = reinterpret_cast<bf16_t*>(&yv);
+            const bf16_t* mh = reinterpret_cast<const bf16_t*>(&bmv);
+#pragma unroll
+            for (int e = 0; e < 8; ++e) yh[e] = bf2f(mh[e]) > 0.f ? yh[e] : (bf16_t)0;
+            *reinterpret_cast<u32x4*>(g.Y + e0) = yv;
+          }
+        }
+      }
+    }
+  }
   if (ct_slot >= 0) CT(ct_slot);
   if constexpr (ACC) {
     if (do_bnr) {
@@ -491,6 +545,9 @@
     }
   }
   if (do_bnr) {
+  int lane_t = lane;
+  asm volatile("" : "+v"(lane_t));
+  const int lc_t = (lane_t % LPR) * 8;
 #pragma unroll
   for (int o = LPR; o < 64; o <<= 1)
 #pragma unroll
@@ -503,16 +560,16 @@
   float* red = smemf;
   lds_barrier();
   if (ct_slot >= 0) CT(ct_slot + 4);
-  if (wr > 0 && lane < LPR)
+  if (wr > 0 && lane_t < LPR)
 #pragma unroll
     for (int e = 0; e < 8; ++e) {
-      float* o = red + ((wr * WN + wc) * TN + lc + e) * 3;
+      float* o = red + ((wr * WN + wc) * TN + lc_t + e) * 3;
       o[0] = sA[e];
       o[1] = sB[e];
       o[2] = sC[e];
     }
   lds_barrier();
-  if (wr != 0 || lane >= LPR || !cok) {
+  if (wr != 0 || lane_t >= LPR || !cok) {
     flush();
     return;
   }
@@ -520,7 +577,7 @@
   for (int e = 0; e < 8; ++e)
 #pragma unroll
     for (int q = 1; q < WM; ++q) {
-      const float* o = red + ((q * WN + wc) * TN + lc + e) * 3;
+      const float* o = red + ((q * WN + wc) * TN + lc_t + e) * 3;
       sA[e] += o[0];
       sB[e] += o[1];
       sC[e] += o[2];
@@ -962,7 +1019,8 @@
     } else {
       __syncthreads();
       CTP(3);
-      conv_epilogue_vec<DGRAD, FM, FN, WM, WN, EWF, decltype(out_row), EpiNone, false, X2>(
+      conv_epilogue_vec<DGRAD, FM, FN, WM, WN, EWF, decltype(out_row), EpiNone, false, X2, EpiNoAcc,
+                        PAR && BM_ == 128 && BN_ == 128 && WM * WN == 8>(
           g, acc, reinterpret_cast<float*>(smem), w, lane, m0, n0, M, (DGRAD && g.bnr_red) ? red_row() : 0l, ty,
           out_row, static_cast<const EpiNone*>(nullptr), ct_slot);
     }
@@ -987,7 +1045,8 @@
           if (!g.Rmask || bf2f(g.Rmask[ri]) > 0.f) v += bf2f(g.R_[ri]);
         }
         const bf16_t h = f2bf(v);
-        g.Y[orow + col] = h;
+        const bool off = DGRAD && g.bnr_red && g.y_masked && !(bf2f(g.bnr_mask[orow + col]) > 0.f);
+        g.Y[orow + col] = off ? (bf16_t)0 : h;
         acc[i][j][r] = bf2f(h);
       }
     }
@@ -1514,7 +1573,17 @@
                               const void* bn_mask, const void* bn_x, const float* bn_ms, float* bn_red,
                               const void* bn_x2, const float* bn_ms2, float* bn_red2, const void* ds_dy,
                               const void* ds_wt_packed, int ds_K, int variant, void* stream) {
+  return mer_conv_dgrad_carry(N, H, W, C, K, R, S, stride, pad, dy, wt_packed, dx, residual, residual_mask, bn_mask,
+                              bn_x, bn_ms, bn_red, bn_x2, bn_ms2, bn_red2, ds_dy, ds_wt_packed, ds_K, 0, variant, stream);
+}
+
+MER_API int mer_conv_dgrad_carry(int N, int H, int W, int C, int K, int R, int S, int stride, int pad, const void* dy,
+                                 const void* wt_packed, void* dx, const void* residual, const void* residual_mask,
+                                 const void* bn_mask, const void* bn_x, const float* bn_ms, float* bn_red,
+                                 const void* bn_x2, const float* bn_ms2, float* bn_red2, const void* ds_dy,
+                                 const void* ds_wt_packed, int ds_K, int store_masked, int variant, void* stream) {
   if (K % 8 || C % 8 || variant < -1 || variant > 7) return (int)hipErrorInvalidValue;
+  if (store_masked && (!bn_red || residual_mask)) return (int)hipErrorInvalidValue;
   if (ds_dy && (stride != 2 || R != 3 || S != 3 || pad != 1 || !ds_wt_packed || ds_K <= 0 || ds_K % 64 || K % 64 ||
                 variant == 0))
     return (int)hipErrorInvalidValue;
@@ -1526,5 +1595,6 @@
   g.bnr_mask = (const bf16_t*)bn_mask; g.bnr_x = (const bf16_t*)bn_x; g.bnr_ms = bn_ms; g.bnr_red = bn_red;
   g.bnr_x2 = (const bf16_t*)bn_x2; g.bnr_ms2 = bn_ms2; g.bnr_red2 = bn_red2;
   g.Wt2 = (const bf16_t*)ds_wt_packed; g.K2 = ds_dy ? ds_K : 0;
+  g.y_masked = store_masked ? 1 : 0;
   return launch_conv_plan<true>(g, conv_plan(g, true, variant), (hipStream_t)stream);
 }
diff --git a/multimodalemotionrecognition_amd/csrc/conv_common.h b/multimodalemotionrecognition_amd/csrc/conv_common.h
--- a/multimodalemotionrecognition_amd/csrc/conv_common.h
+++ b/multimodalemotionrecognition_amd/csrc/conv_common.h
@@ -67,6 +67,7 @@
   const bf16_t* bnr_x2;
   const float* bnr_ms2;
   float* bnr_red2;
+  int y_masked;
   int vec;
   const bf16_t* X2;
   const bf16_t* Wt2;
diff --git a/multimodalemotionrecognition_amd/kernels.py b/multimodalemotionrecognition_amd/kernels.py
--- a/multimodalemotionrecognition_amd/kernels.py
+++ b/multimodalemotionrecognition_amd/kernels.py
@@ -470,7 +470,8 @@
     return r
 
 
-def conv_dgrad(dy, wt, dx, R, S, stride, pad, residual=None, mask=None, variant=-1, bnr=None, ds=None):
+def conv_dgrad(dy, wt, dx, R, S, stride, pad, residual=None, mask=None, variant=-1, bnr=None, ds=None,
+               store_masked=False):
     N, H, W, C = dx.shape
     Kc = dy.shape[-1]
     Ho, Wo = (H + 2 * pad - R) // stride + 1, (W + 2 * pad - S) // stride + 1
@@ -488,6 +489,12 @@
         Kd = ddy.shape[-1]
         if tuple(ddy.shape) != (N, Ho, Wo, Kd) or tuple(dwt.shape) != (C, Kd) or stride != 2 or R != 3 or pad != 1:
             raise ValueError("conv_dgrad ds: a 1x1 / stride-2 downsample gradient beside a 3x3 / stride-2 / pad-1 conv")
+    if store_masked:
+        _launch("conv_dgrad", (N, H, W, C, Kc, R, stride), "mer_conv_dgrad_carry", N, H, W, C, Kc, R, S, stride, pad,
+                dy.data_ptr(), wt.data_ptr(), dx.data_ptr(), _ptr(residual), _ptr(mask), *[_ptr(t) for t in b],
+                _ptr(ds[0] if ds is not None else None), _ptr(ds[1] if ds is not None else None),
+                ds[0].shape[-1] if ds is not None else 0, 1, int(variant), stream_ptr())
+    elif ds is not None:
         _launch("conv_dgrad", (N, H, W, C, Kc, R, stride), "mer_conv_dgrad_ds", N, H, W, C, Kc, R, S, stride, pad,
                 dy.data_ptr(), wt.data_ptr(), dx.data_ptr(), _ptr(residual), _ptr(mask), *[_ptr(t) for t in b],
                 ddy.data_ptr(), dwt.data_ptr(), Kd, int(variant), stream_ptr())
@@ -680,9 +687,9 @@
                   batch_stats=True):
     C = x.shape[-1]
     for t in (dy, mask, x2, dx, dx2):
-        if tuple(t.shape) != tuple(x.shape):
+        if t is not None and tuple(t.shape) != tuple(x.shape):
             raise ValueError("bn_bwd_apply2 tensors must share one shape")
-    LIB("mer_bn_bwd_apply2", x.numel() // C, C, dy.data_ptr(), mask.data_ptr(), x.data_ptr(), ms.data_ptr(),
+    LIB("mer_bn_bwd_apply2", x.numel() // C, C, dy.data_ptr(), _ptr(mask), x.data_ptr(), ms.data_ptr(),
         gamma.data_ptr(), red.data_ptr(), x2.data_ptr(), ms2.data_ptr(), gamma2.data_ptr(), red2.data_ptr(),
         int(batch_stats), dx.data_ptr(), dx2.data_ptr(), _ptr(dgamma), _ptr(dbeta), _ptr(dgamma2), _ptr(dbeta2),
         stream_ptr())
@@ -720,9 +727,14 @@
     LIB("mer_avgpool_fwd", N, H * W, C, x.data_ptr(), y.data_ptr(), stream_ptr())
 
 
-def avgpool_bwd(dy, dx):
+def avgpool_bwd(dy, dx, mask=None):
     N, H, W, C = dx.shape
-    LIB("mer_avgpool_bwd", N, H * W, C, dy.data_ptr(), dx.data_ptr(), stream_ptr())
+    if mask is None:
+        LIB("mer_avgpool_bwd", N, H * W, C, dy.data_ptr(), dx.data_ptr(), stream_ptr())
+        return
+    if tuple(mask.shape) != tuple(dx.shape) or mask.dtype != dx.dtype or not mask.is_contiguous():
+        raise ValueError("avgpool_bwd mask must match dx")
+    LIB("mer_avgpool_bwd_masked", N, H * W, C, dy.data_ptr(), mask.data_ptr(), dx.data_ptr(), stream_ptr())
 
 
 def softmax_avg_fwd(za, zv, out, pa, pv):
diff --git a/multimodalemotionrecognition_amd/video.py b/multimodalemotionrecognition_amd/video.py
--- a/multimodalemotionrecognition_amd/video.py
+++ b/multimodalemotionrecognition_amd/video.py
@@ -491,6 +491,7 @@
 BN_FIN_PAIR = True
 FOLD_EVERY = 2
 FUSED_DS_DGRAD = True
+MASK_CARRY = True
 
 
 class _WgradLane:
@@ -508,7 +509,7 @@
 
 @torch.no_grad()
 def block_backward(trunk, blk: BasicBlock, sv, dx: torch.Tensor, grads, training: bool = True, pre=None,
-                   prev=None, arena=None, lane=None, bidx=None):
+                   prev=None, arena=None, lane=None, bidx=None, carry=False):
     dev = dx.device
     xin, bc1, bms1, ba1, bc2, bms2, cd, msd, out = sv
     if arena is None:
@@ -517,6 +518,7 @@
     if own_lane:
         lane = _WgradLane(dev)
     g_out = dx
+    m_out = None if carry else out
     s = blk.stride
     C2 = bc2.shape[-1]
     if pre is not None:
@@ -529,49 +531,52 @@
                 if cd is not None else None
     else:
         red2 = arena.take(C2, parts=1)
-        K.bn_bwd_reduce(g_out, out, bc2, bms2, red2, arena.take(C2, parts=K.BN_RED_WS_ROWS))
+        K.bn_bwd_reduce(g_out, m_out, bc2, bms2, red2, arena.take(C2, parts=K.BN_RED_WS_ROWS))
         redd = None
         if cd is not None:
             redd = arena.take(C2, parts=1)
-            K.bn_bwd_reduce(g_out, out, cd, msd, redd, arena.take(C2, parts=K.BN_RED_WS_ROWS))
+            K.bn_bwd_reduce(g_out, m_out, cd, msd, redd, arena.take(C2, parts=K.BN_RED_WS_ROWS))
     if cd is not None and BN_BWD_PAIR:
         dc2, dcd = torch.empty_like(bc2), torch.empty_like(cd)
         bd = blk.downsample[1]
-        K.bn_bwd_apply2(g_out, out, bc2, bms2, blk.bn2.weight, red2, dc2, _grad(blk.bn2.weight, grads),
+        K.bn_bwd_apply2(g_out, m_out, bc2, bms2, blk.bn2.weight, red2, dc2, _grad(blk.bn2.weight, grads),
                         _grad(blk.bn2.bias, grads), cd, msd, bd.weight, redd, dcd, _grad(bd.weight, grads),
                         _grad(bd.bias, grads), training)
     else:
-        dc2 = _bn_bwd(g_out, out, bc2, bms2, blk.bn2, red2, grads, training)
-        dcd = _bn_bwd(g_out, out, cd, msd, blk.downsample[1], redd, grads, training) if cd is not None else None
+        dc2 = _bn_bwd(g_out, m_out, bc2, bms2, blk.bn2, red2, grads, training)
+        dcd = _bn_bwd(g_out, m_out, cd, msd, blk.downsample[1], redd, grads, training) if cd is not None else None
     w2 = _grad(blk.conv2.weight, grads)
     if w2 is not None:
         lane.run(lambda: K.conv_wgrad(ba1, dc2, w2, 3, 3, 1, 1, defer=lane.folds), ba1, dc2, w2, block=bidx)
     da1 = torch.empty_like(ba1)
     C1 = bc1.shape[-1]
     red1p = arena.take(C1, parts=K.bn_red_rows(ba1.numel() // C1))
-    rows1 = K.conv_dgrad(dc2, trunk.packed(blk.conv2, C2, True), da1, 3, 3, 1, 1, bnr=(ba1, bc1, bms1, red1p))
+    rows1 = K.conv_dgrad(dc2, trunk.packed(blk.conv2, C2, True), da1, 3, 3, 1, 1, bnr=(ba1, bc1, bms1, red1p),
+                         store_masked=carry)
     red1 = K.partials_sum(red1p, torch.empty(C1, 2, device=dev, dtype=torch.float32), rows1)
-    dc1 = _bn_bwd(da1, ba1, bc1, bms1, blk.bn1, red1, grads, training)
+    dc1 = _bn_bwd(da1, None if carry else ba1, bc1, bms1, blk.bn1, red1, grads, training)
     w1 = _grad(blk.conv1.weight, grads)
     if w1 is not None:
         lane.run(lambda: K.conv_wgrad(xin, dc1, w1, 3, 3, s, 1, defer=lane.folds), xin, dc1, w1, block=bidx)
     dxin = torch.empty_like(xin)
     Cin = xin.shape[-1]
     bnr, nxt = _bnr_target(prev[0], prev[1], arena) if prev is not None else (None, None)
+    sm = carry and bnr is not None
     if cd is not None:
         wd = _grad(blk.downsample[0].weight, grads)
         if wd is not None:
             lane.run(lambda: K.conv_wgrad(xin, dcd, wd, 1, 1, s, 0, defer=lane.folds), xin, dcd, wd, block=bidx)
         if FUSED_DS_DGRAD and s == 2:
             rows = K.conv_dgrad(dc1, trunk.packed(blk.conv1, Cin, True), dxin, 3, 3, s, 1, bnr=bnr,
-                                ds=(dcd, trunk.packed(blk.downsample[0], Cin, True)))
+                                ds=(dcd, trunk.packed(blk.downsample[0], Cin, True)), store_masked=sm)
         else:
             dxd = torch.empty_like(xin)
             K.conv_dgrad(dcd, trunk.packed(blk.downsample[0], Cin, True), dxd, 1, 1, s, 0)
-            rows = K.conv_dgrad(dc1, trunk.packed(blk.conv1, Cin, True), dxin, 3, 3, s, 1, residual=dxd, bnr=bnr)
+            rows = K.conv_dgrad(dc1, trunk.packed(blk.conv1, Cin, True), dxin, 3, 3, s, 1, residual=dxd, bnr=bnr,
+                                store_masked=sm)
     else:
-        rows = K.conv_dgrad(dc1, trunk.packed(blk.conv1, Cin, True), dxin, 3, 3, s, 1, residual=g_out, mask=out,
-                            bnr=bnr)
+        rows = K.conv_dgrad(dc1, trunk.packed(blk.conv1, Cin, True), dxin, 3, 3, s, 1, residual=g_out, mask=m_out,
+                            bnr=bnr, store_masked=sm)
     if own_lane:
         lane.join()
     return dxin, (nxt + (rows,) if nxt is not None else None)
@@ -594,7 +599,7 @@
         dev = dfeat.device
         x = saved["final"]
         dx = torch.empty_like(x)
-        K.avgpool_bwd(dfeat, dx)
+        K.avgpool_bwd(dfeat, dx, mask=x if MASK_CARRY else None)
         svs = saved["blocks"]
         arena = _StatsArena(trunk, dev, floats=sum(_block_bwd_floats(sv) for sv in svs) + 2 * K.BN_RED_WS_ROWS * 64 * 2)
         state = dict(dx=dx, pre=None, grads={}, arena=arena, i=len(svs) - 1, lane=_WgradLane(dev))
@@ -610,7 +615,7 @@
         prev = (svs[i - 1], blocks[i - 1]) if i > 0 else None
         state["dx"], state["pre"] = block_backward(trunk, blocks[i], svs[i], state["dx"], state["grads"], training,
                                                    pre=state["pre"], prev=prev, arena=state["arena"],
-                                                   lane=state["lane"], bidx=i)
+                                                   lane=state["lane"], bidx=i, carry=MASK_CARRY)
         if FOLD_EVERY and i % FOLD_EVERY == 0 and i > 0:
             state["lane"].join()
         state["i"] = i - 1
```

New measurement: 225.1 steps/s (median of 6 runs). About the same (+0.8%).
